# XiandaGuo/OpenStereo

Hardware: NVIDIA H100
Metric: stereo_pairs_per_sec_gwcnet_256x512_d192 (higher is better)
Workload: dtype f32

## Files before the change

openstereo_b200/csrc/conv3d_tc.cu:

```cuda
#include <cstdlib>
#include <type_traits>

#include "tc_common.cuh"

namespace osb {

constexpr int TC_W = 128;
constexpr int TC_KC = 32;
constexpr int TC_TILES = TC_WGS;
constexpr int TC_ROWS = TC_TILES + 2;
constexpr int TC_STAGES = 4;
constexpr int TC_RAW = 2;
constexpr int TC_ROW_BYTES = TC_W * TC_KC * 4;
constexpr int TC_PC = 16;

struct TcParams {
  const float* x;
  const void* w;
  const float* scale;
  const float* shift;
  const float* residual;
  float* y;
  int B, D, H, Cin, Cout;
  int act;
  float kappa;
  unsigned int* overflow;
  int out_ndhwc, res_ndhwc;
  int bulk_rows;
  int in_ncdhw;
  int items, hblocks;
};

template <int COUT>
struct TcCfg {
  static constexpr int N3 = 3 * COUT;
  static constexpr int B_SLICE = N3 * TC_KC * 4;
  static constexpr int NPASS = COUT / TC_PC;
  static constexpr int LD = 3 * TC_PC + 4;
  static constexpr int XCHG_FLOATS = 6 * 2 * TC_PC;
  static constexpr int A_OFF = 0;
  static constexpr int B_OFF = A_OFF + TC_STAGES * TC_ROW_BYTES;
  static constexpr int RAW_OFF = B_OFF + TC_BSLOTS * 3 * B_SLICE;
  static constexpr int STAGE_OFF = RAW_OFF + TC_RAW * TC_ROW_BYTES;
  static constexpr int BAR_OFF = STAGE_OFF + TC_WGS * 128 * LD * 4;
  static constexpr size_t SMEM = 1024 + (size_t)BAR_OFF + 256 + TC_WGS * XCHG_FLOATS * 4 + 2 * COUT * 4;
  static_assert(COUT % TC_PC == 0, "the epilogue stages whole passes of TC_PC channels");
  static_assert(B_SLICE % 1024 == 0, "weight slices must stay 1024-byte aligned");
  static_assert(32 * LD >= TP_WARP_FLOATS, "store_ndhwc_chunk32 transposes through the warp's own rows of the staging tile");
  static_assert(SMEM <= 232448, "shared memory budget of one CTA exceeded");
};

template <int COUT>
__device__ __forceinline__ void tc_stage_pass(float* stage, const float (&acc)[2][3 * COUT / 2], int pass, int wq, int lane) {
  constexpr int LD = TcCfg<COUT>::LD;
#pragma unroll
  for (int h = 0; h < 2; ++h) {
    float* r0 = stage + (64 * h + 16 * wq + (lane >> 2)) * LD + 2 * (lane & 3);
#pragma unroll
    for (int kw = 0; kw < 3; ++kw)
#pragma unroll
      for (int jj = 0; jj < TC_PC / 8; ++jj) {
        const int j = (kw * COUT + pass * TC_PC) / 8 + jj;
        *reinterpret_cast<float2*>(r0 + TC_PC * kw + 8 * jj) = make_float2(acc[h][4 * j], acc[h][4 * j + 1]);
        *reinterpret_cast<float2*>(r0 + 8 * LD + TC_PC * kw + 8 * jj) = make_float2(acc[h][4 * j + 2], acc[h][4 * j + 3]);
      }
  }
}

template <int COUT>
__global__ void __launch_bounds__(TC_WG_THREADS, 1) conv3d_tc_kernel(const TcParams p) {
  using C = TcCfg<COUT>;
  constexpr int N3 = C::N3;
  constexpr int B_SLICE = C::B_SLICE;
  extern __shared__ __align__(1024) uint8_t smem_raw[];
  uint8_t* smem = smem_raw + ((1024u - (smem_u32(smem_raw) & 1023u)) & 1023u);
  uint8_t* a_buf = smem + C::A_OFF;
  uint8_t* b_buf = smem + C::B_OFF;
  uint8_t* raw_buf = smem + C::RAW_OFF;
  float* stage = reinterpret_cast<float*>(smem + C::STAGE_OFF);
  uint64_t* bars = reinterpret_cast<uint64_t*>(smem + C::BAR_OFF);
  uint64_t* a_ready = bars;
  uint64_t* a_empty = a_ready + TC_STAGES;
  uint64_t* b_full = a_empty + TC_STAGES;
  uint64_t* b_empty = b_full + TC_BSLOTS * 3;
  uint64_t* raw_full = b_empty + TC_BSLOTS * 3;
  uint64_t* raw_empty = raw_full + TC_RAW;
  float* xchg = reinterpret_cast<float*>(smem + C::BAR_OFF + 256);
  float* s_scale = xchg + TC_WGS * C::XCHG_FLOATS;
  float* s_shift = s_scale + COUT;

  const int warp = threadIdx.x >> 5, lane = threadIdx.x & 31;
  const int nchunk = p.Cin / TC_KC;

  if (threadIdx.x == 0) {
    for (int s = 0; s < TC_STAGES; ++s) {
      mbar_init(&a_ready[s], 128);
      mbar_init(&a_empty[s], 4 * TC_WGS);
    }
    for (int k = 0; k < TC_BSLOTS * 3; ++k) {
      mbar_init(&b_full[k], 1);
      mbar_init(&b_empty[k], 4 * TC_WGS);
    }
    for (int k = 0; k < TC_RAW; ++k) {
      mbar_init(&raw_full[k], 1);
      mbar_init(&raw_empty[k], 128);
    }
    fence_mbar_init();
  }
  for (int c = threadIdx.x; c < COUT; c += blockDim.x) {
    s_scale[c] = p.scale ? p.scale[c] : 1.f;
    s_shift[c] = p.shift ? p.shift[c] : 0.f;
  }
  for (int i = threadIdx.x; i < TC_WGS * C::XCHG_FLOATS; i += blockDim.x) xchg[i] = 0.f;
  __syncthreads();
  struct RowIter {
    int it, kd, ch, r;
  };
  auto advance = [&](RowIter& s) {
    for (;;) {
      if (s.it >= p.items) return false;
      if (++s.r < TC_ROWS) return true;
      s.r = -1;
      if (++s.ch < nchunk) continue;
      s.ch = 0;
      const int d = (s.it / p.hblocks) % p.D;
      for (++s.kd; s.kd < 3; ++s.kd) {
        const int din = d + s.kd - 1;
        if (din >= 0 && din < p.D) break;
      }
      if (s.kd < 3) continue;
      s.it += gridDim.x;
      if (s.it >= p.items) return false;
      const int d2 = (s.it / p.hblocks) % p.D;
      s.kd = (d2 == 0) ? 1 : 0;
    }
  };
  if (warp < 4 * TC_WGS) {
    setmaxnreg_inc<TC_CONSUMER_REGS>();
    const int wg = warp >> 2;
    stage += wg * 128 * C::LD;
    xchg += wg * C::XCHG_FLOATS;
    const int bar_stage = 1 + 2 * wg, bar_xchg = 2 + 2 * wg;
    constexpr uint32_t LO = TcK<TC_KC>::LO_OFF;
    constexpr uint32_t A_HALF = 64 * TC_KC * 4 / 16;
    const uint64_t dbase = desc_sw128_base();
    const uint32_t b16 = (smem_u32(b_buf) & 0x3FFFF) >> 4;
    const int q = warp & 3;
    const int m = q * 32 + lane;
    uint32_t rowc = 0, phc = 0;
    for (int it = blockIdx.x; it < p.items; it += gridDim.x) {
      const int d = (it / p.hblocks) % p.D;
      float acc[2][N3 / 2];
      uint32_t accum = 0;
      for (int kd = 0; kd < 3; ++kd) {
        const int din = d + kd - 1;
        if (din < 0 || din >= p.D) continue;
        for (int ch = 0; ch < nchunk; ++ch, ++phc) {
          const uint32_t bslot = (phc & 1) * 3;
#pragma unroll
          for (int r = 0; r < TC_ROWS; ++r) {
            const uint32_t s = rowc % TC_STAGES, par = (rowc / TC_STAGES) & 1;
            mbar_wait(&a_ready[s], par);
            const int kh = r - wg;
            if (kh >= 0 && kh < 3) {
              mbar_wait(&b_full[bslot + kh], (phc >> 1) & 1);
              const uint64_t da0 = dbase | (uint64_t)((smem_u32(a_buf + s * TC_ROW_BYTES) & 0x3FFFF) >> 4);
              const uint64_t db0 = dbase | (uint64_t)(b16 + (bslot + kh) * (B_SLICE / 16));
              wg_fence();
#pragma unroll
              for (int ks = 0; ks < TcK<TC_KC>::KSTEPS; ++ks)
                wg_mma_split<N3>(acc, da0 + 2 * ks, A_HALF, db0 + 2 * ks, LO, ks > 0 ? 1u : accum);
              wg_commit();
              wg_wait_all();
              accum = 1;
              wg_release(&b_empty[bslot + kh], lane);
            }
            wg_release(&a_empty[s], lane);
            ++rowc;
          }
        }
      }
      const int h = (it % p.hblocks) * TC_TILES + wg;
      if (h >= p.H) continue;
      const float corr = 1.f + p.kappa * (float)(((d > 0) + 1 + (d + 1 < p.D)) * nchunk * 3 * TcK<TC_KC>::KSTEPS * 3);
      float out[COUT];
#pragma unroll
      for (int pass = 0; pass < C::NPASS; ++pass) {
        named_bar_sync(bar_stage, 128);
        tc_stage_pass<COUT>(stage, acc, pass, q, lane);
        named_bar_sync(bar_stage, 128);
        const float* srow = stage + m * C::LD;
        float* xq = xchg + (q + 1) * 2 * TC_PC;
        if (lane == 31) {
#pragma unroll
          for (int i = 0; i < TC_PC; i += 4)
            *reinterpret_cast<float4*>(xq + i) = *reinterpret_cast<const float4*>(srow + i);
        }
        if (lane == 0) {
#pragma unroll
          for (int i = 0; i < TC_PC; i += 4)
            *reinterpret_cast<float4*>(xq + TC_PC + i) = *reinterpret_cast<const float4*>(srow + 2 * TC_PC + i);
        }
        named_bar_sync(bar_xchg, 128);
        const float* xl = xq - 2 * TC_PC;
        const float* xr = xq + 3 * TC_PC;
#pragma unroll
        for (int i0 = 0; i0 < TC_PC; i0 += 4) {
          const float4 l4 = *reinterpret_cast<const float4*>(xl + i0);
          const float4 r4 = *reinterpret_cast<const float4*>(xr + i0);
          const float4 p04 = *reinterpret_cast<const float4*>(srow + i0);
          const float4 p14 = *reinterpret_cast<const float4*>(srow + TC_PC + i0);
          const float4 p24 = *reinterpret_cast<const float4*>(srow + 2 * TC_PC + i0);
          const float le[4] = {l4.x, l4.y, l4.z, l4.w}, re[4] = {r4.x, r4.y, r4.z, r4.w};
          const float p0[4] = {p04.x, p04.y, p04.z, p04.w}, p1[4] = {p14.x, p14.y, p14.z, p14.w}, p2[4] = {p24.x, p24.y, p24.z, p24.w};
#pragma unroll
          for (int k = 0; k < 4; ++k) {
            float left = __shfl_up_sync(0xffffffffu, p0[k], 1);
            float right = __shfl_down_sync(0xffffffffu, p2[k], 1);
            left = (lane == 0) ? le[k] : left;
            right = (lane == 31) ? re[k] : right;
            out[pass * TC_PC + i0 + k] = ((left + p1[k]) + right) * corr;
          }
        }
      }
      const int b = it / (p.hblocks * p.D);
      const size_t vox = (((size_t)b * p.D + d) * p.H + h) * TC_W + m;
      const size_t plane = (size_t)p.D * p.H * TC_W;
      const size_t ncdhw0 = (size_t)b * p.Cout * plane + ((size_t)d * p.H + h) * TC_W + m;
      if constexpr (COUT == 32) {
        if (p.out_ndhwc && (!p.residual || p.res_ndhwc)) {
          store_ndhwc_chunk32(stage + q * 32 * C::LD, lane, out, p.y + (vox - lane) * COUT,
                              p.residual ? p.residual + (vox - lane) * COUT : nullptr, COUT, s_scale, s_shift, p.act);
          continue;
        }
      }
#pragma unroll
      for (int i = 0; i < COUT; ++i) out[i] = fmaf(out[i], s_scale[i], s_shift[i]);
      if (p.residual) {
        if (p.res_ndhwc) {
          const float4* rp = reinterpret_cast<const float4*>(p.residual + vox * COUT);
#pragma unroll
          for (int i = 0; i < COUT / 4; ++i) {
            const float4 rv = __ldg(rp + i);
            out[4 * i] += rv.x, out[4 * i + 1] += rv.y, out[4 * i + 2] += rv.z, out[4 * i + 3] += rv.w;
          }
        } else {
#pragma unroll
          for (int i = 0; i < COUT; ++i)
            if (i < p.Cout) out[i] += __ldg(p.residual + ncdhw0 + (size_t)i * plane);
        }
      }
      if (p.act == OSB_ACT_RELU) {
#pragma unroll
        for (int i = 0; i < COUT; ++i) out[i] = fmaxf(out[i], 0.f);
      } else if (p.act == OSB_ACT_LEAKY) {
#pragma unroll
        for (int i = 0; i < COUT; ++i) out[i] = out[i] > 0.f ? out[i] : 0.01f * out[i];
      }
      if (p.out_ndhwc) {
        float4* yp = reinterpret_cast<float4*>(p.y + vox * COUT);
#pragma unroll
        for (int i = 0; i < COUT / 4; ++i) yp[i] = make_float4(out[4 * i], out[4 * i + 1], out[4 * i + 2], out[4 * i + 3]);
      } else {
#pragma unroll
        for (int i = 0; i < COUT; ++i)
          if (i < p.Cout) p.y[ncdhw0 + (size_t)i * plane] = out[i];
      }
    }
  }
  else if (warp < 4 * TC_WGS + 4) {
    setmaxnreg_dec<TC_LOADER_REGS>();
    const int lt = threadIdx.x - 4 * TC_WGS * 32;
    const int vsel = lt >> 3, c16 = lt & 7;
    const int vcol = ((vsel & 1) << 2) | ((vsel >> 1) & 3) | (vsel & 8);
    float amax = 0.f;
    auto run = [&](auto in_ncdhw) {
      constexpr bool NCDHW = decltype(in_ncdhw)::value;
      const size_t row_stride = (size_t)TC_W * p.Cin;
      auto load_row = [&](const RowIter& s, float4 (&v)[8]) {
        const int hb = s.it % p.hblocks;
        const int d = (s.it / p.hblocks) % p.D;
        const int b = s.it / (p.hblocks * p.D);
        const int hin = hb * TC_TILES - 1 + s.r, din = d + s.kd - 1;
        if (hin >= 0 && hin < p.H && NCDHW) {
          const size_t plane = (size_t)p.D * p.H * TC_W;
          const float* src = p.x + (((size_t)b * p.Cin + s.ch * TC_KC) * p.D + din) * p.H * TC_W + (size_t)hin * TC_W + lt;
#pragma unroll
          for (int j = 0; j < 8; ++j, src += 4 * plane)
            v[j] = make_float4(__ldg(src), __ldg(src + plane), __ldg(src + 2 * plane), __ldg(src + 3 * plane));
          const bool swap = (lt >> 3) & 1;
#pragma unroll
          for (int j = 0; j < 8; j += 2) {
            const float4 e = v[j], o = v[j + 1];
            v[j] = swap ? o : e;
            v[j + 1] = swap ? e : o;
          }
        } else if (hin >= 0 && hin < p.H) {
          const float* src = p.x + (((size_t)b * p.D + din) * p.H + hin) * row_stride + s.ch * TC_KC + c16 * 4 + vcol * p.Cin;
#pragma unroll
          for (int j = 0; j < 8; ++j) v[j] = __ldg(reinterpret_cast<const float4*>(src + 16 * j * p.Cin));
        } else {
#pragma unroll
          for (int j = 0; j < 8; ++j) v[j] = make_float4(0.f, 0.f, 0.f, 0.f);
        }
      };
      uint32_t rowc = 0;
      auto store_row = [&](const float4 (&v)[8]) {
        const uint32_t s = rowc % TC_STAGES, par = (rowc / TC_STAGES) & 1;
        mbar_wait_relaxed(&a_empty[s], par ^ 1);
        uint8_t* tile = a_buf + s * TC_ROW_BYTES;
        if (NCDHW) {
#pragma unroll
          for (int j = 0; j < 8; ++j) stage_f16_split<TC_KC>(tile, lt, j ^ ((lt >> 3) & 1), v[j], amax);
        } else {
#pragma unroll
          for (int j = 0; j < 8; ++j) stage_f16_split<TC_KC>(tile, vcol + 16 * j, c16, v[j], amax);
        }
        fence_proxy_async();
        mbar_arrive(&a_ready[s]);
        ++rowc;
      };
      RowIter ld{(int)blockIdx.x, 0, 0, -1};
      if (ld.it < p.items) ld.kd = (((ld.it / p.hblocks) % p.D) == 0) ? 1 : 0;
      if (p.bulk_rows) {
        uint32_t rawc = 0;
        while (advance(ld)) {
          const int hb = ld.it % p.hblocks;
          const int hin = hb * TC_TILES - 1 + ld.r;
          const uint32_t slot = rawc % TC_RAW, par = (rawc / TC_RAW) & 1;
          mbar_wait_relaxed(&raw_full[slot], par);
          float4 v[8];
          if (hin >= 0 && hin < p.H && NCDHW) {
            const float* src = reinterpret_cast<const float*>(raw_buf + slot * TC_ROW_BYTES) + lt;
#pragma unroll
            for (int j = 0; j < 8; ++j) {
              const float* q = src + 4 * (j ^ ((lt >> 3) & 1)) * TC_W;
              v[j] = make_float4(q[0], q[TC_W], q[2 * TC_W], q[3 * TC_W]);
            }
          } else if (hin >= 0 && hin < p.H) {
            const float* src = reinterpret_cast<const float*>(raw_buf + slot * TC_ROW_BYTES) + c16 * 4;
#pragma unroll
            for (int j = 0; j < 8; ++j) v[j] = *reinterpret_cast<const float4*>(src + (vcol + 16 * j) * TC_KC);
          } else {
#pragma unroll
            for (int j = 0; j < 8; ++j) v[j] = make_float4(0.f, 0.f, 0.f, 0.f);
          }
          store_row(v);
          mbar_arrive(&raw_empty[slot]);
          ++rawc;
        }
        tc_report_overflow(p.overflow, amax);
        amax = 0.f;
      }
      float4 va[8], vb[8];
      bool has_a = !p.bulk_rows && advance(ld);
      if (has_a) load_row(ld, va);
      bool has_b = has_a && advance(ld);
      if (has_b) load_row(ld, vb);
      while (has_a) {
        store_row(va);
        has_a = has_b && advance(ld);
        if (has_a) load_row(ld, va);
        if (!has_b) break;
        store_row(vb);
        has_b = has_a && advance(ld);
        if (has_b) load_row(ld, vb);
      }
      tc_report_overflow(p.overflow, amax);
    };
    if (p.in_ncdhw) run(std::true_type{});
    else run(std::false_type{});
  }
  else {
    setmaxnreg_dec<TC_PRODUCER_REGS>();
    if (warp == 4 * TC_WGS + 4 && elect_one()) {
      const uint8_t* wsrc = reinterpret_cast<const uint8_t*>(p.w);
      uint32_t phc = 0;
      for (int it = blockIdx.x; it < p.items; it += gridDim.x) {
        const int d = (it / p.hblocks) % p.D;
        for (int kd = 0; kd < 3; ++kd) {
          const int din = d + kd - 1;
          if (din < 0 || din >= p.D) continue;
          for (int ch = 0; ch < nchunk; ++ch, ++phc) {
            for (int kh = 0; kh < 3; ++kh) {
              const uint32_t slot = (phc & 1) * 3 + kh;
              const size_t slice = ((size_t)kd * nchunk + ch) * 3 + kh;
              mbar_wait_relaxed(&b_empty[slot], ((phc >> 1) & 1) ^ 1);
              mbar_arrive_expect_tx(&b_full[slot], B_SLICE);
              bulk_g2s(b_buf + slot * B_SLICE, wsrc + slice * B_SLICE, B_SLICE, &b_full[slot]);
            }
          }
        }
      }
    }
    else if (warp == 4 * TC_WGS + 5 && p.bulk_rows && elect_one()) {
      RowIter ld{(int)blockIdx.x, 0, 0, -1};
      if (ld.it < p.items) ld.kd = (((ld.it / p.hblocks) % p.D) == 0) ? 1 : 0;
      uint32_t rawc = 0;
      while (advance(ld)) {
        const int hb = ld.it % p.hblocks;
        const int d = (ld.it / p.hblocks) % p.D;
        const int b = ld.it / (p.hblocks * p.D);
        const int hin = hb * TC_TILES - 1 + ld.r, din = d + ld.kd - 1;
        const uint32_t slot = rawc % TC_RAW, par = (rawc / TC_RAW) & 1;
        mbar_wait_relaxed(&raw_empty[slot], par ^ 1);
        if (hin >= 0 && hin < p.H && p.in_ncdhw) {
          const size_t plane = (size_t)p.D * p.H * TC_W;
          const float* src = p.x + (((size_t)b * p.Cin + ld.ch * TC_KC) * p.D + din) * p.H * TC_W + (size_t)hin * TC_W;
          mbar_arrive_expect_tx(&raw_full[slot], TC_ROW_BYTES);
          for (int c = 0; c < TC_KC; ++c)
            bulk_g2s(raw_buf + slot * TC_ROW_BYTES + c * (TC_W * 4), src + c * plane, TC_W * 4, &raw_full[slot]);
        } else if (hin >= 0 && hin < p.H) {
          const float* src = p.x + (((size_t)b * p.D + din) * p.H + hin) * (size_t)(TC_W * TC_KC);
          mbar_arrive_expect_tx(&raw_full[slot], TC_ROW_BYTES);
          bulk_g2s(raw_buf + slot * TC_ROW_BYTES, src, TC_ROW_BYTES, &raw_full[slot]);
        } else {
          mbar_arrive(&raw_full[slot]);
        }
        ++rawc;
      }
    }
    __syncwarp();
  }
}

__global__ void __launch_bounds__(256) ncdhw_to_ndhwc_kernel(const float* __restrict__ x, float* __restrict__ y, int C, int Cp,
                                                             size_t vol) {
  __shared__ float tile[32][33];
  const int b = blockIdx.z;
  const size_t v0 = (size_t)blockIdx.x * 32;
  const int c0 = blockIdx.y * 32;
  const int tx = threadIdx.x & 31, ty = threadIdx.x >> 5;
  for (int i = ty; i < 32; i += 8) {
    const int c = c0 + i;
    const size_t v = v0 + tx;
    tile[i][tx] = (c < C && v < vol) ? __ldg(x + ((size_t)b * C + c) * vol + v) : 0.f;
  }
  __syncthreads();
  for (int i = ty; i < 32; i += 8) {
    const size_t v = v0 + i;
    const int c = c0 + tx;
    if (c < Cp && v < vol) y[((size_t)b * vol + v) * Cp + c] = tile[tx][i];
  }
}

template <int COUT>
static int launch_tc(const TcParams& p, cudaStream_t stream) {
  const size_t smem = TcCfg<COUT>::SMEM;
  auto kernel = conv3d_tc_kernel<COUT>;
  static PerDeviceFlag configured;
  if (!configured.here()) {
    cudaError_t e = cudaFuncSetAttribute(kernel, cudaFuncAttributeMaxDynamicSharedMemorySize, (int)smem);
    if (e != cudaSuccess) {
      set_error("conv3d_tc: cannot reserve %zu bytes of shared memory: %s", smem, cudaGetErrorString(e));
      return OSB_ECUDA;
    }
    configured.here() = true;
  }
  const int sms = sm_count();
  const int grid = (int)cap_persistent_grid(p.items < sms ? p.items : sms);
  static const std::string variant = tc_variant_name("tc<%d>", COUT);
  set_tc_variant(variant.c_str());
  kernel<<<grid, TC_WG_THREADS, smem, stream>>>(p);
  count_launch();
  return check_launch("conv3d_tc_kernel");
}

int launch_tcg_dispatch(const float* x, const void* w, const float* scale, const float* shift, const float* residual, float* y,
                        int B, int Cin, int Cout, int D, int H, int W, int act, int out_ndhwc, int res_ndhwc, cudaStream_t stream,
                        const float* gate = nullptr, int ystride = 0);
int launch_tcg_dilated2(const float* x, const void* w, const float* scale, const float* shift, const float* residual, float* y,
                        int B, int Cin, int Cout, int H, int W, int act, int out_ndhwc, int res_ndhwc, cudaStream_t stream);

}

extern "C" {

int osb_tc_general_width(int W) { return W >= OSB_TC_MIN_WIDTH ? 1 : 0; }

int osb_conv3d_tc_kc(int Cin, int Cout, int W, int stride) {
  if (stride != 1) return 0;
  if (W == osb::TC_W && (Cout == 32 || (Cout >= 1 && Cout <= 16)) && Cin % 32 == 0 && Cin >= 32) return 32;
  if (Cin % 16 == 0 && Cin >= 16 &&
      ((W == 64 && Cout == 64) || (W == 32 && (Cout == 64 || Cout == 96 || Cout == 128)) || (W == 16 && (Cout == 64 || Cout == 96)) ||
       (W == osb::TC_W && (Cout == 64 || Cout == 128))))
    return 16;
  if (Cin % 16 == 0 && Cin >= 16 && osb_tc_general_width(W) && (Cout == 32 || Cout == 64 || Cout == 128))
    return 16;
  return 0;
}

int osb_conv3d_tc_supported(int Cin, int Cout, int W, int stride) { return osb_conv3d_tc_kc(Cin, Cout, W, stride) != 0; }

int osb_ncdhw_to_ndhwc_pad(const float* x, float* y, int B, int C, int Cpad, int D, int H, int W, osb_stream_t stream) {
  using namespace osb;
  OSB_REQUIRE(x && y, "ncdhw_to_ndhwc: null pointer");
  OSB_REQUIRE(B > 0 && C > 0 && Cpad >= C && D > 0 && H > 0 && W > 0 && B <= 65535, "ncdhw_to_ndhwc: bad shape");
  const size_t vol = (size_t)D * H * W;
  dim3 grid((unsigned)((vol + 31) / 32), (Cpad + 31) / 32, B);
  ncdhw_to_ndhwc_kernel<<<grid, 256, 0, (cudaStream_t)stream>>>(x, y, C, Cpad, vol);
  count_launch();
  return check_launch("ncdhw_to_ndhwc_kernel");
}

int osb_ncdhw_to_ndhwc(const float* x, float* y, int B, int C, int D, int H, int W, osb_stream_t stream) {
  return osb_ncdhw_to_ndhwc_pad(x, y, B, C, C, D, H, W, stream);
}

static int conv3d_k3_tc_impl(const float* x_ndhwc, const void* w_split, const float* scale, const float* shift,
                             const float* residual, float* y, int B, int Cin, int Cout, int D, int H, int W, int act,
                             int out_ndhwc, int res_ndhwc, int in_ncdhw, osb_stream_t stream, const float* gate = nullptr,
                             int ystride = 0) {
  using namespace osb;
  OSB_REQUIRE(x_ndhwc && w_split && y, "conv3d_k3_tc: null pointer");
  OSB_REQUIRE(B > 0 && D > 0 && H > 0, "conv3d_k3_tc: empty shape");
  OSB_REQUIRE(osb_conv3d_tc_supported(Cin, Cout, W, 1), "conv3d_k3_tc: unsupported shape Cin=%d Cout=%d W=%d", Cin, Cout, W);
  OSB_REQUIRE(act >= 0 && act <= 2, "conv3d_k3_tc: unknown activation %d", act);
  OSB_REQUIRE((reinterpret_cast<uintptr_t>(x_ndhwc) & 15) == 0 && (reinterpret_cast<uintptr_t>(w_split) & 15) == 0 &&
                  (reinterpret_cast<uintptr_t>(y) & 15) == 0 && (reinterpret_cast<uintptr_t>(residual) & 15) == 0,
              "conv3d_k3_tc: pointers must be 16-byte aligned");
  OSB_REQUIRE(!in_ncdhw || osb_conv3d_tc_kc(Cin, Cout, W, 1) == 32, "conv3d_k3_tc: NCDHW input is served by the W = 128 kernel only");
  OSB_REQUIRE(ystride == 0 || (ystride >= Cout && ystride % 4 == 0 && osb_conv3d_tc_kc(Cin, Cout, W, 1) == 16 && out_ndhwc &&
                                (!residual || res_ndhwc)),
              "conv3d_k3_tc: a channel slice (ystride %d) needs channels-last tensors on the 16-channel-chunk kernels", ystride);
  OSB_REQUIRE(!gate || (osb_conv3d_tc_kc(Cin, Cout, W, 1) == 16 && out_ndhwc && (!residual || res_ndhwc) &&
                        (reinterpret_cast<uintptr_t>(gate) & 15) == 0),
              "conv3d_k3_tc: the gate operand needs a channels-last output (and residual) on the 16-channel-chunk kernels");
  if (osb_conv3d_tc_kc(Cin, Cout, W, 1) == 16)
    return launch_tcg_dispatch(x_ndhwc, w_split, scale, shift, residual, y, B, Cin, Cout, D, H, W, act, out_ndhwc, res_ndhwc,
                               (cudaStream_t)stream, gate, ystride);
  TcParams p{};
  p.x = x_ndhwc, p.w = w_split, p.scale = scale, p.shift = shift, p.residual = residual, p.y = y;
  p.B = B, p.D = D, p.H = H, p.Cin = Cin, p.Cout = Cout, p.act = act;
  p.kappa = rz_kappa(), p.overflow = tc_overflow_flag();
  OSB_REQUIRE(p.overflow, "conv3d_k3_tc: cannot allocate the overflow flag");
  p.out_ndhwc = out_ndhwc, p.res_ndhwc = res_ndhwc, p.in_ncdhw = in_ncdhw;
  {
    static const int bulk = [] { const char* e = getenv("OSB_TC_BULK"); return e ? atoi(e) : 1; }();
    p.bulk_rows = (bulk && (in_ncdhw || Cin == TC_KC)) ? 1 : 0;
  }
  p.hblocks = (H + TC_TILES - 1) / TC_TILES;
  const long long items = (long long)B * D * p.hblocks;
  OSB_REQUIRE(items < (1ll << 31), "conv3d_k3_tc: too many work items");
  p.items = (int)items;
  if (Cout <= 16) {
    OSB_REQUIRE(!out_ndhwc && (!residual || !res_ndhwc), "conv3d_k3_tc: Cout <= 16 writes (and adds) NCDHW tensors only");
    return launch_tc<16>(p, (cudaStream_t)stream);
  }
  return launch_tc<32>(p, (cudaStream_t)stream);
}

int osb_conv3d_k3_tc_fwd(const float* x_ndhwc, const void* w_split, const float* scale, const float* shift,
                         const float* residual, float* y, int B, int Cin, int Cout, int D, int H, int W, int act,
                         int out_ndhwc, int res_ndhwc, osb_stream_t stream) {
  return conv3d_k3_tc_impl(x_ndhwc, w_split, scale, shift, residual, y, B, Cin, Cout, D, H, W, act, out_ndhwc, res_ndhwc, 0, stream);
}

int osb_conv3d_k3_tc_gate_fwd(const float* x_ndhwc, const void* w_split, const float* scale, const float* shift,
                              const float* residual, const float* gate_nhwc, float* y, int B, int Cin, int Cout, int D, int H, int W,
                              int act, osb_stream_t stream) {
  OSB_REQUIRE(gate_nhwc, "conv3d_k3_tc_gate: null gate");
  return conv3d_k3_tc_impl(x_ndhwc, w_split, scale, shift, residual, y, B, Cin, Cout, D, H, W, act, 1, 1, 0, stream, gate_nhwc);
}

int osb_conv3d_k3_tc_cs_fwd(const float* x_ndhwc, const void* w_split, const float* scale, const float* shift, const float* residual,
                            const float* gate_nhwc, float* y, int B, int Cin, int Cout, int D, int H, int W, int act, int ystride,
                            osb_stream_t stream) {
  return conv3d_k3_tc_impl(x_ndhwc, w_split, scale, shift, residual, y, B, Cin, Cout, D, H, W, act, 1, 1, 0, stream, gate_nhwc, ystride);
}

int osb_conv3d_k3_tc_ncdhw_fwd(const float* x_ncdhw, const void* w_split, const float* scale, const float* shift,
                               const float* residual, float* y, int B, int Cin, int Cout, int D, int H, int W, int act,
                               int out_ndhwc, int res_ndhwc, osb_stream_t stream) {
  return conv3d_k3_tc_impl(x_ncdhw, w_split, scale, shift, residual, y, B, Cin, Cout, D, H, W, act, out_ndhwc, res_ndhwc, 1, stream);
}

int osb_conv2d_tc_kc(int Cin, int Cout, int W, int dilation) {
  if (dilation == 1) return osb_conv3d_tc_kc(Cin, Cout, W, 1);
  if (dilation == 2 && W == osb::TC_W && Cout == 128 && Cin % 16 == 0 && Cin >= 16) return 16;
  return 0;
}

int osb_conv2d_k3_tc_fwd(const float* x_nhwc, const void* w_split, const float* scale, const float* shift, const float* residual,
                         float* y, int B, int Cin, int Cout, int H, int W, int dilation, int act, int out_nhwc, int res_nhwc,
                         osb_stream_t stream) {
  using namespace osb;
  if (dilation == 1)
    return osb_conv3d_k3_tc_fwd(x_nhwc, w_split, scale, shift, residual, y, B, Cin, Cout, 1, H, W, act, out_nhwc, res_nhwc, stream);
  OSB_REQUIRE(x_nhwc && w_split && y, "conv2d_k3_tc: null pointer");
  OSB_REQUIRE(B > 0 && H > 0, "conv2d_k3_tc: empty shape");
  OSB_REQUIRE(osb_conv2d_tc_kc(Cin, Cout, W, dilation) != 0, "conv2d_k3_tc: unsupported shape Cin=%d Cout=%d W=%d dilation=%d", Cin, Cout,
              W, dilation);
  OSB_REQUIRE(act >= 0 && act <= 2, "conv2d_k3_tc: unknown activation %d", act);
  OSB_REQUIRE((reinterpret_cast<uintptr_t>(x_nhwc) & 15) == 0 && (reinterpret_cast<uintptr_t>(w_split) & 15) == 0 &&
                  (reinterpret_cast<uintptr_t>(y) & 15) == 0 && (reinterpret_cast<uintptr_t>(residual) & 15) == 0,
              "conv2d_k3_tc: pointers must be 16-byte aligned");
  return launch_tcg_dilated2(x_nhwc, w_split, scale, shift, residual, y, B, Cin, Cout, H, W, act, out_nhwc, res_nhwc,
                             (cudaStream_t)stream);
}
}
```

openstereo_b200/csrc/conv3d_tcg.cu:

```cuda
#include "tc_common.cuh"

namespace osb {

struct TcgParams {
  const float* x;
  const void* w;
  const float* scale;
  const float* shift;
  const float* residual;
  const float* gate;
  float* y;
  int B, D, H, Cin;
  int act;
  float kappa;
  unsigned int* overflow;
  int out_ndhwc, res_ndhwc;
  int items, hblocks;
  int Wr, ctiles;
  int ystride;
};

template <int COUT, int KC, int W, int TILES, int DIL = 1, bool GW = false>
struct TcgCfg {
  static_assert(!GW || W == 128, "general-width tiles are 128-column segments of one image row");
  static constexpr int HALO = GW ? DIL : 0;
  static constexpr int CSTEP = 128 - 2 * HALO;
  static_assert(DIL == 1 || (W == 128 && DIL == 2 && COUT >= 64), "dilation 2 is instantiated for full-width rows only");
  static constexpr int R = 128 / W;
  static constexpr int ROWB = KC * 4;
  static constexpr int UNIT_BYTES = 128 * ROWB;
  static constexpr int N3 = 3 * COUT;
  static constexpr int G = 32;
  static constexpr int NG = COUT / G;
  static constexpr int NG3 = 3 * G;
  static constexpr int B_SLICE = N3 * ROWB;
  static constexpr int B_SUB = NG3 * ROWB;
  static constexpr int LD = NG3 + 4;
  static constexpr int NT = TC_WGS * TILES;
  static constexpr int TS = R * DIL;
  static constexpr int HSPAN = NT * TS;
  __host__ __device__ static constexpr int row0(int hb) { return (hb / DIL) * HSPAN + (hb % DIL) * R; }
  __host__ static int hblocks(int H) { return DIL * ((H + HSPAN - 1) / HSPAN); }
  static constexpr int NLW = 4;
  static constexpr int XCHG_FLOATS = 2 * 4 * 2 * DIL * 32;
  static constexpr int FIXED_SMEM = 1024 + TC_BSLOTS * 3 * B_SUB + TC_WGS * 128 * LD * 4 + 1024 + TC_WGS * XCHG_FLOATS * 4 + 3 * COUT * 4;
  static constexpr int STAGES = (232448 - FIXED_SMEM) / UNIT_BYTES < 10 ? (232448 - FIXED_SMEM) / UNIT_BYTES : 10;
  static_assert(STAGES >= NLW, "the ring must hold at least one unit per loader warp");
  static constexpr int S_FIRST = -DIL;
  static constexpr int S_LAST = (NT - 1) * TS + DIL;
  static constexpr int KSTEPS = KC / 16;
  static constexpr int LO = KC / 8;
  static constexpr int A_OFF = 0;
  static constexpr int B_OFF = A_OFF + STAGES * UNIT_BYTES;
  static constexpr int STAGE_OFF = B_OFF + TC_BSLOTS * 3 * B_SUB;
  static constexpr int BAR_OFF = STAGE_OFF + TC_WGS * 128 * LD * 4;
  static constexpr int THREADS = TC_WG_THREADS;
  static constexpr size_t SMEM = 1024 + (size_t)BAR_OFF + 1024 + TC_WGS * XCHG_FLOATS * 4 + 3 * COUT * 4;
  static_assert(SMEM <= 232448, "shared memory budget of one CTA exceeded");
  static_assert(TILES == 1, "a consumer warpgroup holds one accumulator tile");
  static_assert(DIL == 1 || R == 1, "interleaved row blocks assume one image row per tile");
  static_assert(COUT % G == 0, "output channels come in groups of 32");
  static_assert(B_SUB % 1024 == 0 && UNIT_BYTES % 1024 == 0, "operand tiles must stay 1024-byte aligned");
  static constexpr int tile_of(int s, int kh) {
    const int num = s - (kh - 1) * DIL;
    return (num >= 0 && num % TS == 0 && num / TS < NT) ? num / TS : -1;
  }
  static constexpr bool used(int s) { return tile_of(s, 0) >= 0 || tile_of(s, 1) >= 0 || tile_of(s, 2) >= 0; }
  static constexpr int units_per_phase() {
    int n = 0;
    for (int s = S_FIRST; s <= S_LAST; ++s) n += used(s) ? 1 : 0;
    return n;
  }
  static constexpr int NU = units_per_phase();
  static constexpr int unit_s(int j) {
    int k = 0;
    for (int s = S_FIRST; s <= S_LAST; ++s)
      if (used(s)) {
        if (k == j) return s;
        ++k;
      }
    return S_LAST;
  }
};

template <int COUT, int KC, int W, int TILES, int DIL = 1, bool GW = false, bool GATE = false>
__global__ void __launch_bounds__(TcgCfg<COUT, KC, W, TILES, DIL, GW>::THREADS, 1) conv3d_tcg_kernel(const TcgParams p) {
  using C = TcgCfg<COUT, KC, W, TILES, DIL, GW>;
  extern __shared__ __align__(1024) uint8_t smem_raw[];
  uint8_t* smem = reinterpret_cast<uint8_t*>((reinterpret_cast<uintptr_t>(smem_raw) + 1023) & ~static_cast<uintptr_t>(1023));
  uint8_t* a_buf = smem + C::A_OFF;
  uint8_t* b_buf = smem + C::B_OFF;
  float* stage = reinterpret_cast<float*>(smem + C::STAGE_OFF);
  uint64_t* bars = reinterpret_cast<uint64_t*>(smem + C::BAR_OFF);
  uint64_t* a_ready = bars;
  uint64_t* a_empty = a_ready + C::STAGES;
  uint64_t* b_full = a_empty + C::STAGES;
  uint64_t* b_empty = b_full + TC_BSLOTS * 3;
  float* xchg = reinterpret_cast<float*>(smem + C::BAR_OFF + 1024);
  float* s_scale = xchg + TC_WGS * C::XCHG_FLOATS;
  float* s_shift = s_scale + COUT;
  float* zeros = s_shift + COUT;

  const int warp = threadIdx.x >> 5, lane = threadIdx.x & 31;
  const int nchunk = p.Cin / KC;
  const int Wp = GW ? p.Wr : W;
  const int YS = (W < 32 && p.ystride) ? p.ystride : COUT;
  const int ctiles = GW ? p.ctiles : 1;

  if (threadIdx.x == 0) {
    for (int s = 0; s < C::STAGES; ++s) {
      mbar_init(&a_ready[s], 32);
      mbar_init(&a_empty[s], 4 * TC_WGS);
    }
    for (int k = 0; k < TC_BSLOTS * 3; ++k) {
      mbar_init(&b_full[k], 1);
      mbar_init(&b_empty[k], 4 * TC_WGS);
    }
    fence_mbar_init();
  }
  for (int c = threadIdx.x; c < COUT; c += blockDim.x) {
    s_scale[c] = p.scale ? p.scale[c] : 1.f;
    s_shift[c] = p.shift ? p.shift[c] : 0.f;
    zeros[c] = 0.f;
  }
  __syncthreads();

  if (warp < 4 * TC_WGS) {
    setmaxnreg_inc<TC_CONSUMER_REGS>();
    const int wg = warp >> 2;
    stage += wg * 128 * C::LD;
    xchg += wg * C::XCHG_FLOATS;
    const int bar_stage = 1 + 2 * wg, bar_xchg = 2 + 2 * wg;
    const uint64_t dbase = (KC == 32) ? desc_sw128_base() : desc_sw64_base();
    constexpr uint32_t A_HALF = 64 * C::ROWB / 16;
    const uint32_t b16 = (smem_u32(b_buf) & 0x3FFFF) >> 4;
    const int q = warp & 3;
    const int m = q * 32 + lane;
    const int rr = m / W, wcol = m % W;
    const bool has_left_q = ((q * 32) % W) != 0;
    const bool has_right_q = (((q + 1) * 32) % W) != 0;
    uint32_t unitc = 0, phc = 0, exc = 0;
    for (int it = blockIdx.x; it < p.items; it += gridDim.x) {
      const int cg = (it % C::NG) * C::G;
      const int it0 = it / C::NG;
      const int ct = it0 % ctiles;
      const int hb = (it0 / ctiles) % p.hblocks;
      const int d = (it0 / (ctiles * p.hblocks)) % p.D;
      const int b = it0 / (ctiles * p.hblocks * p.D);
      {
        float acc[2][C::NG3 / 2];
        uint32_t accum = 0;
        for (int kd = 0; kd < 3; ++kd) {
          const int din = d + kd - 1;
          if (din < 0 || din >= p.D) continue;
          for (int ch = 0; ch < nchunk; ++ch, ++phc) {
#pragma unroll
            for (int s = C::S_FIRST; s <= C::S_LAST; ++s) {
              if (!C::used(s)) continue;
              const uint32_t slot = unitc % C::STAGES, par = (unitc / C::STAGES) & 1;
              mbar_wait(&a_ready[slot], par);
              const uint64_t da0 = dbase | (uint64_t)((smem_u32(a_buf + slot * C::UNIT_BYTES) & 0x3FFFF) >> 4);
#pragma unroll
              for (int kh = 0; kh < 3; ++kh) {
                if (C::tile_of(s, kh) != wg) continue;
                const uint32_t bslot = (phc & 1) * 3 + kh;
                mbar_wait(&b_full[bslot], (phc >> 1) & 1);
                const uint64_t db0 = dbase | (uint64_t)(b16 + (bslot * C::B_SUB) / 16);
                wg_fence();
#pragma unroll
                for (int ks = 0; ks < C::KSTEPS; ++ks)
                  wg_mma_split<C::NG3>(acc, da0 + 2 * ks, A_HALF, db0 + 2 * ks, C::LO, ks > 0 ? 1u : accum);
                wg_commit();
                wg_wait_all();
                accum = 1;
                wg_release(&b_empty[bslot], lane);
              }
              wg_release(&a_empty[slot], lane);
              ++unitc;
            }
          }
        }
        named_bar_sync(bar_stage, 128);
        wg_stage<C::NG3>(stage, C::LD, acc, q, lane);
        named_bar_sync(bar_stage, 128);
      }
      const int col = GW ? ct * C::CSTEP - C::HALO + m : wcol;
      const bool cvalid = !GW || (m >= C::HALO && m < 128 - C::HALO && col < Wp);
      const uint32_t vmask = GW ? __ballot_sync(0xffffffffu, cvalid) : 0xffffffffu;
      const float corr = 1.f + p.kappa * (float)(((d > 0) + 1 + (d + 1 < p.D)) * nchunk * 3 * C::KSTEPS * 3);
      {
        const int h = C::row0(hb) + wg * C::TS + rr;
        const bool live = h < p.H;
        const ptrdiff_t vox = (((ptrdiff_t)b * p.D + d) * p.H + h) * Wp + col;
        if (live && cvalid && p.residual && p.res_ndhwc) {
          const float* rp = p.residual + vox * YS;
#pragma unroll
          for (int k = 0; k < COUT; k += 32) asm volatile("prefetch.global.L2 [%0];" ::"l"(rp + k));
        }
        const size_t plane = (size_t)p.D * p.H * Wp;
        const ptrdiff_t ncdhw0 = (ptrdiff_t)b * COUT * plane + ((ptrdiff_t)d * p.H + h) * Wp + col;
        {
          const float* srow = stage + m * C::LD;
          float* xb = xchg + (exc & 1) * (4 * 2 * DIL * 32);
          ++exc;
          if (lane >= 32 - DIL) {
#pragma unroll
            for (int i = 0; i < 32; i += 4)
              *reinterpret_cast<float4*>(xb + ((q * 2) * DIL + lane - (32 - DIL)) * 32 + i) = *reinterpret_cast<const float4*>(srow + i);
          }
          if (lane < DIL) {
#pragma unroll
            for (int i = 0; i < 32; i += 4)
              *reinterpret_cast<float4*>(xb + ((q * 2 + 1) * DIL + lane) * 32 + i) = *reinterpret_cast<const float4*>(srow + 2 * C::G + i);
          }
          named_bar_sync(bar_xchg, 128);
          const float* xl = has_left_q ? xb + (((q - 1) * 2) * DIL + (lane < DIL ? lane : 0)) * 32 : zeros;
          const float* xr = has_right_q ? xb + (((q + 1) * 2 + 1) * DIL + (lane >= 32 - DIL ? lane - (32 - DIL) : 0)) * 32 : zeros;
          float out[32];
#pragma unroll
          for (int i0 = 0; i0 < 32; i0 += 4) {
            const float4 l4 = *reinterpret_cast<const float4*>(xl + i0);
            const float4 r4 = *reinterpret_cast<const float4*>(xr + i0);
            const float4 p04 = *reinterpret_cast<const float4*>(srow + i0);
            const float4 p14 = *reinterpret_cast<const float4*>(srow + C::G + i0);
            const float4 p24 = *reinterpret_cast<const float4*>(srow + 2 * C::G + i0);
            const float le[4] = {l4.x, l4.y, l4.z, l4.w}, re[4] = {r4.x, r4.y, r4.z, r4.w};
            const float p0[4] = {p04.x, p04.y, p04.z, p04.w}, p1[4] = {p14.x, p14.y, p14.z, p14.w}, p2[4] = {p24.x, p24.y, p24.z, p24.w};
#pragma unroll
            for (int k = 0; k < 4; ++k) {
              const int i = i0 + k;
              float left = __shfl_up_sync(0xffffffffu, p0[k], DIL);
              float right = __shfl_down_sync(0xffffffffu, p2[k], DIL);
              left = (lane < DIL) ? le[k] : left;
              right = (lane >= 32 - DIL) ? re[k] : right;
              if (W < 32) {
                left = (wcol < DIL) ? 0.f : left;
                right = (wcol >= W - DIL) ? 0.f : right;
              }
              out[i] = ((left + p1[k]) + right) * corr;
            }
          }
          const uint32_t vm = (W < 32) ? __ballot_sync(0xffffffffu, live) : (live ? vmask : 0u);
          if (vm && p.out_ndhwc && (!p.residual || p.res_ndhwc)) {
            const ptrdiff_t gvox = GATE ? ((ptrdiff_t)b * p.H + h) * Wp + col - lane : 0;
            store_ndhwc_chunk32(stage + q * 32 * C::LD, lane, out, p.y + (vox - lane) * YS + cg,
                                p.residual ? p.residual + (vox - lane) * YS + cg : nullptr, YS, s_scale + cg, s_shift + cg, p.act,
                                vm, (GATE && p.gate) ? p.gate + gvox * YS + cg : nullptr);
          } else if (live && cvalid) {
#pragma unroll
            for (int i = 0; i < 32; ++i) out[i] = fmaf(out[i], s_scale[cg + i], s_shift[cg + i]);
            if (p.residual) {
              if (p.res_ndhwc) {
                const float4* rp = reinterpret_cast<const float4*>(p.residual + vox * YS + cg);
#pragma unroll
                for (int i = 0; i < 8; ++i) {
                  const float4 rv = __ldg(rp + i);
                  out[4 * i] += rv.x, out[4 * i + 1] += rv.y, out[4 * i + 2] += rv.z, out[4 * i + 3] += rv.w;
                }
              } else {
#pragma unroll
                for (int i = 0; i < 32; ++i) out[i] += __ldg(p.residual + ncdhw0 + (size_t)(cg + i) * plane);
              }
            }
            if (p.act == OSB_ACT_RELU) {
#pragma unroll
              for (int i = 0; i < 32; ++i) out[i] = fmaxf(out[i], 0.f);
            } else if (p.act == OSB_ACT_LEAKY) {
#pragma unroll
              for (int i = 0; i < 32; ++i) out[i] = out[i] > 0.f ? out[i] : 0.01f * out[i];
            }
            if (p.out_ndhwc) {
              float4* yp = reinterpret_cast<float4*>(p.y + vox * YS + cg);
#pragma unroll
              for (int i = 0; i < 8; ++i) yp[i] = make_float4(out[4 * i], out[4 * i + 1], out[4 * i + 2], out[4 * i + 3]);
            } else {
#pragma unroll
              for (int i = 0; i < 32; ++i) p.y[ncdhw0 + (size_t)(cg + i) * plane] = out[i];
            }
          }
        }
      }
    }
  }
  else if (warp < 4 * TC_WGS + C::NLW) {
    setmaxnreg_dec<TC_LOADER_REGS>();
    const int lw = warp - 4 * TC_WGS;
    static_assert(KC == 16, "lane_voxel / unit-row mapping below is written for 64-byte operand rows");
    constexpr int CPR = KC / 4;
    constexpr int VPL = 32 / CPR;
    constexpr int NLD = 128 / VPL;
    static_assert(W % VPL == 0, "a load instruction must not straddle image rows");
    const int v0 = lane_voxel<KC>(lane), c = lane % CPR;
    float amax = 0.f;
    uint32_t ubase = 0;
    int first = lw;
    auto fill = [&](const float* base, size_t rstride, size_t cstride, int h_first, int h_step, uint32_t u, int col0) {
      float4 v[NLD];
#pragma unroll
      for (int j = 0; j < NLD; ++j) {
        const int hin = h_first + h_step * ((VPL * j) / W);
        const size_t off = (size_t)((VPL * j) / W) * rstride + (size_t)((VPL * j) % W) * cstride;
        bool ok = hin >= 0 && hin < p.H;
        if (GW) ok = ok && (unsigned)(col0 + VPL * j) < (unsigned)Wp;
        v[j] = ok ? __ldg(reinterpret_cast<const float4*>(base + (ptrdiff_t)off)) : make_float4(0.f, 0.f, 0.f, 0.f);
      }
      const uint32_t slot = u % C::STAGES, ph = (u / C::STAGES) & 1;
      mbar_wait_relaxed(&a_empty[slot], ph ^ 1);
      uint8_t* tile = a_buf + slot * C::UNIT_BYTES;
#pragma unroll
      for (int j = 0; j < NLD; ++j) stage_f16_split<KC>(tile, v0 + VPL * j, c, v[j], amax);
      fence_proxy_async();
      mbar_arrive(&a_ready[slot]);
    };
    for (int it = blockIdx.x; it < p.items; it += gridDim.x) {
      const int it0 = it / C::NG;
      const int ct = it0 % ctiles;
      const int hb = (it0 / ctiles) % p.hblocks;
      const int d = (it0 / (ctiles * p.hblocks)) % p.D;
      const int b = it0 / (ctiles * p.hblocks * p.D);
      const int h0 = C::row0(hb);
      const int col0 = ct * C::CSTEP - C::HALO + v0;
      for (int kd = 0; kd < 3; ++kd) {
        const int din = d + kd - 1;
        if (din < 0 || din >= p.D) continue;
        const float* plane = p.x + ((size_t)b * p.D + din) * p.H * (size_t)Wp * p.Cin;
        for (int ch = 0; ch < nchunk; ++ch) {
#pragma unroll 1
          for (int j = first; j < C::NU; j += C::NLW) {
            const int s = C::unit_s(j);
            const float* base = plane + ((ptrdiff_t)(h0 + s) * Wp + col0) * p.Cin + ch * KC + c * 4;
            fill(base, (size_t)Wp * p.Cin, (size_t)p.Cin, h0 + s, 1, ubase + j, col0);
          }
          ubase += C::NU;
          first = (first + C::NLW - C::NU % C::NLW) % C::NLW;
        }
      }
    }
    tc_report_overflow(p.overflow, amax);
  }
  else {
    setmaxnreg_dec<TC_PRODUCER_REGS>();
    if (warp == 4 * TC_WGS + C::NLW && elect_one()) {
      const uint8_t* wsrc = reinterpret_cast<const uint8_t*>(p.w);
      uint32_t phc = 0;
      for (int it = blockIdx.x; it < p.items; it += gridDim.x) {
        const int cg = (it % C::NG) * C::G;
        const int d = (it / C::NG / (ctiles * p.hblocks)) % p.D;
        for (int kd = 0; kd < 3; ++kd) {
          const int din = d + kd - 1;
          if (din < 0 || din >= p.D) continue;
          for (int ch = 0; ch < nchunk; ++ch, ++phc) {
            for (int kh = 0; kh < 3; ++kh) {
              const uint32_t slot = (phc & 1) * 3 + kh;
              const size_t slice = ((size_t)kd * nchunk + ch) * 3 + kh;
              mbar_wait_relaxed(&b_empty[slot], ((phc >> 1) & 1) ^ 1);
              mbar_arrive_expect_tx(&b_full[slot], C::B_SUB);
#pragma unroll
              for (int kw = 0; kw < 3; ++kw)
                bulk_g2s(b_buf + slot * C::B_SUB + kw * C::G * C::ROWB, wsrc + slice * C::B_SLICE + (size_t)(kw * COUT + cg) * C::ROWB,
                         C::G * C::ROWB, &b_full[slot]);
            }
          }
        }
      }
    }
    __syncwarp();
  }
}

template <int COUT, int KC, int W, int TILES, int DIL = 1, bool GW = false, bool GATE = false>
static int launch_tcg(TcgParams& p, cudaStream_t stream) {
  using C = TcgCfg<COUT, KC, W, TILES, DIL, GW>;
  auto kernel = conv3d_tcg_kernel<COUT, KC, W, TILES, DIL, GW, GATE>;
  if (!GATE && p.gate) {
    set_error("conv3d_tcg: no gated instantiation for Cout=%d W=%d", COUT, W);
    return OSB_EUNSUPPORTED;
  }
  if (W >= 32 && p.ystride && p.ystride != COUT) {
    set_error("conv3d_tcg: channel slices are instantiated for W = 16 only");
    return OSB_EUNSUPPORTED;
  }
  static PerDeviceFlag configured;
  if (!configured.here()) {
    cudaError_t e = cudaFuncSetAttribute(kernel, cudaFuncAttributeMaxDynamicSharedMemorySize, (int)C::SMEM);
    if (e != cudaSuccess) {
      set_error("conv3d_tcg: cannot reserve %zu bytes of shared memory: %s", C::SMEM, cudaGetErrorString(e));
      return OSB_ECUDA;
    }
    configured.here() = true;
  }
  p.hblocks = C::hblocks(p.H);
  if (GW) p.ctiles = (p.Wr + C::CSTEP - 1) / C::CSTEP;
  else p.Wr = W, p.ctiles = 1;
  const long long items = (long long)p.B * p.D * p.hblocks * p.ctiles * C::NG;
  OSB_REQUIRE(items < (1ll << 31), "conv3d_tcg: too many work items");
  p.items = (int)items;
  const int sms = sm_count();
  const int grid = (int)cap_persistent_grid(p.items < sms ? p.items : sms);
  static const std::string variant = tc_variant_name("tcg<%d,%d,%d,%d,%d,%d,%d>", COUT, KC, W, TILES, DIL, (int)GW, (int)GATE);
  set_tc_variant(variant.c_str());
  kernel<<<grid, C::THREADS, C::SMEM, stream>>>(p);
  count_launch();
  cudaError_t le = cudaGetLastError();
  if (le != cudaSuccess) {
    cudaFuncAttributes fa{};
    (void)cudaFuncGetAttributes(&fa, kernel);
    set_error("conv3d_tcg_kernel<%d,%d,%d,%d>: launch failed: %s (threads %d, kernel maxThreadsPerBlock %d, regs %d, static smem %zu, "
              "dynamic smem %zu, max dynamic %d)", COUT, KC, W, TILES, cudaGetErrorString(le), C::THREADS, fa.maxThreadsPerBlock,
              fa.numRegs, fa.sharedSizeBytes, C::SMEM, fa.maxDynamicSharedSizeBytes);
    return OSB_ECUDA;
  }
  return OSB_OK;
}

int launch_tcg_dispatch(const float* x, const void* w, const float* scale, const float* shift, const float* residual, float* y,
                        int B, int Cin, int Cout, int D, int H, int W, int act, int out_ndhwc, int res_ndhwc, cudaStream_t stream,
                        const float* gate, int ystride) {
  TcgParams p{};
  p.x = x, p.w = w, p.scale = scale, p.shift = shift, p.residual = residual, p.y = y, p.gate = gate;
  p.ystride = ystride;
  p.B = B, p.D = D, p.H = H, p.Cin = Cin, p.act = act, p.out_ndhwc = out_ndhwc, p.res_ndhwc = res_ndhwc;
  p.kappa = rz_kappa(), p.overflow = tc_overflow_flag();
  if (!p.overflow) return OSB_ECUDA;
  if (Cin % 16 != 0 || Cin < 16) return -1;
  if (W == 64 && Cout == 64 && gate) return launch_tcg<64, 16, 64, 1, 1, false, true>(p, stream);
  if (W == 32 && Cout == 96 && gate) return launch_tcg<96, 16, 32, 1, 1, false, true>(p, stream);
  if (W == 64 && Cout == 64) return launch_tcg<64, 16, 64, 1>(p, stream);
  if (W == 32 && Cout == 64) return launch_tcg<64, 16, 32, 1>(p, stream);
  if (W == 32 && Cout == 128) return launch_tcg<128, 16, 32, 1>(p, stream);
  if (W == 32 && Cout == 96) return launch_tcg<96, 16, 32, 1>(p, stream);
  if (W == 16 && Cout == 96) return launch_tcg<96, 16, 16, 1, 1, false, true>(p, stream);
  if (W == 16 && Cout == 64) return launch_tcg<64, 16, 16, 1, 1, false, true>(p, stream);
  if (W == 128 && Cout == 64) return launch_tcg<64, 16, 128, 1>(p, stream);
  if (W == 128 && Cout == 128) return launch_tcg<128, 16, 128, 1>(p, stream);
  p.Wr = W;
  if (Cout == 32) return launch_tcg<32, 16, 128, 1, 1, true>(p, stream);
  if (Cout == 64) return launch_tcg<64, 16, 128, 1, 1, true>(p, stream);
  if (Cout == 128) return launch_tcg<128, 16, 128, 1, 1, true>(p, stream);
  return -1;
}

int launch_tcg_dilated2(const float* x, const void* w, const float* scale, const float* shift, const float* residual, float* y,
                        int B, int Cin, int Cout, int H, int W, int act, int out_ndhwc, int res_ndhwc, cudaStream_t stream) {
  TcgParams p{};
  p.x = x, p.w = w, p.scale = scale, p.shift = shift, p.residual = residual, p.y = y;
  p.B = B, p.D = 1, p.H = H, p.Cin = Cin, p.act = act, p.out_ndhwc = out_ndhwc, p.res_ndhwc = res_ndhwc;
  p.kappa = rz_kappa(), p.overflow = tc_overflow_flag();
  if (!p.overflow) return OSB_ECUDA;
  if (Cin % 16 != 0 || Cin < 16) return -1;
  if (W == 128 && Cout == 128) return launch_tcg<128, 16, 128, 1, 2>(p, stream);
  return -1;
}

}
```

openstereo_b200/csrc/tc_common.cuh:

```cuda
#pragma once
#include "common.cuh"

namespace osb {

__device__ __forceinline__ void mbar_wait_relaxed(uint64_t* bar, uint32_t parity) {
  uint32_t done;
  for (;;) {
    asm volatile(
        "{\n.reg .pred p;\nmbarrier.try_wait.parity.shared::cta.b64 p, [%1], %2;\nselp.u32 %0, 1, 0, p;\n}\n"
        : "=r"(done)
        : "r"(smem_u32(bar)), "r"(parity)
        : "memory");
    if (done) return;
    __nanosleep(64);
  }
}
__device__ __forceinline__ void mbar_arrive(uint64_t* bar) {
  asm volatile("mbarrier.arrive.shared::cta.b64 _, [%0];" ::"r"(smem_u32(bar)) : "memory");
}
__device__ __forceinline__ uint64_t desc_sw128_base() {
  uint64_t d = 0;
  d |= (uint64_t)1 << 16;
  d |= (uint64_t)(1024 >> 4) << 32;
  d |= (uint64_t)1 << 62;
  return d;
}
__device__ __forceinline__ uint64_t desc_sw64_base() {
  uint64_t d = 0;
  d |= (uint64_t)1 << 16;
  d |= (uint64_t)(512 >> 4) << 32;
  d |= (uint64_t)2 << 62;
  return d;
}

template <int N>
__device__ __forceinline__ void wgmma_f16(float (&d)[N / 2], uint64_t da, uint64_t db, uint32_t accumulate);
template <>
__device__ __forceinline__ void wgmma_f16<32>(float (&d)[16], uint64_t da, uint64_t db, uint32_t accumulate) {
  asm volatile(
      "{\n.reg .pred p;\nsetp.ne.b32 p, %18, 0;\n"
      "wgmma.mma_async.sync.aligned.m64n32k16.f32.f16.f16 {%0, %1, %2, %3, %4, %5, %6, %7, %8, %9, %10, %11, %12, %13, %14, %15}, %16, %17, p, 1, 1, 0, 0;\n}\n"
      : "+f"(d[0]), "+f"(d[1]), "+f"(d[2]), "+f"(d[3]), "+f"(d[4]), "+f"(d[5]), "+f"(d[6]), "+f"(d[7]), "+f"(d[8]), "+f"(d[9]), "+f"(d[10]), "+f"(d[11]), "+f"(d[12]), "+f"(d[13]), "+f"(d[14]), "+f"(d[15])
      : "l"(da), "l"(db), "r"(accumulate)
      : "memory");
}

template <>
__device__ __forceinline__ void wgmma_f16<48>(float (&d)[24], uint64_t da, uint64_t db, uint32_t accumulate) {
  asm volatile(
      "{\n.reg .pred p;\nsetp.ne.b32 p, %26, 0;\n"
      "wgmma.mma_async.sync.aligned.m64n48k16.f32.f16.f16 {%0, %1, %2, %3, %4, %5, %6, %7, %8, %9, %10, %11, %12, %13, %14, %15, %16, %17, %18, %19, %20, %21, %22, %23}, %24, %25, p, 1, 1, 0, 0;\n}\n"
      : "+f"(d[0]), "+f"(d[1]), "+f"(d[2]), "+f"(d[3]), "+f"(d[4]), "+f"(d[5]), "+f"(d[6]), "+f"(d[7]), "+f"(d[8]), "+f"(d[9]), "+f"(d[10]), "+f"(d[11]), "+f"(d[12]), "+f"(d[13]), "+f"(d[14]), "+f"(d[15]), "+f"(d[16]), "+f"(d[17]), "+f"(d[18]), "+f"(d[19]), "+f"(d[20]), "+f"(d[21]), "+f"(d[22]), "+f"(d[23])
      : "l"(da), "l"(db), "r"(accumulate)
      : "memory");
}

template <>
__device__ __forceinline__ void wgmma_f16<64>(float (&d)[32], uint64_t da, uint64_t db, uint32_t accumulate) {
  asm volatile(
      "{\n.reg .pred p;\nsetp.ne.b32 p, %34, 0;\n"
      "wgmma.mma_async.sync.aligned.m64n64k16.f32.f16.f16 {%0, %1, %2, %3, %4, %5, %6, %7, %8, %9, %10, %11, %12, %13, %14, %15, %16, %17, %18, %19, %20, %21, %22, %23, %24, %25, %26, %27, %28, %29, %30, %31}, %32, %33, p, 1, 1, 0, 0;\n}\n"
      : "+f"(d[0]), "+f"(d[1]), "+f"(d[2]), "+f"(d[3]), "+f"(d[4]), "+f"(d[5]), "+f"(d[6]), "+f"(d[7]), "+f"(d[8]), "+f"(d[9]), "+f"(d[10]), "+f"(d[11]), "+f"(d[12]), "+f"(d[13]), "+f"(d[14]), "+f"(d[15]), "+f"(d[16]), "+f"(d[17]), "+f"(d[18]), "+f"(d[19]), "+f"(d[20]), "+f"(d[21]), "+f"(d[22]), "+f"(d[23]), "+f"(d[24]), "+f"(d[25]), "+f"(d[26]), "+f"(d[27]), "+f"(d[28]), "+f"(d[29]), "+f"(d[30]), "+f"(d[31])
      : "l"(da), "l"(db), "r"(accumulate)
      : "memory");
}

template <>
__device__ __forceinline__ void wgmma_f16<96>(float (&d)[48], uint64_t da, uint64_t db, uint32_t accumulate) {
  asm volatile(
      "{\n.reg .pred p;\nsetp.ne.b32 p, %50, 0;\n"
      "wgmma.mma_async.sync.aligned.m64n96k16.f32.f16.f16 {%0, %1, %2, %3, %4, %5, %6, %7, %8, %9, %10, %11, %12, %13, %14, %15, %16, %17, %18, %19, %20, %21, %22, %23, %24, %25, %26, %27, %28, %29, %30, %31, %32, %33, %34, %35, %36, %37, %38, %39, %40, %41, %42, %43, %44, %45, %46, %47}, %48, %49, p, 1, 1, 0, 0;\n}\n"
      : "+f"(d[0]), "+f"(d[1]), "+f"(d[2]), "+f"(d[3]), "+f"(d[4]), "+f"(d[5]), "+f"(d[6]), "+f"(d[7]), "+f"(d[8]), "+f"(d[9]), "+f"(d[10]), "+f"(d[11]), "+f"(d[12]), "+f"(d[13]), "+f"(d[14]), "+f"(d[15]), "+f"(d[16]), "+f"(d[17]), "+f"(d[18]), "+f"(d[19]), "+f"(d[20]), "+f"(d[21]), "+f"(d[22]), "+f"(d[23]), "+f"(d[24]), "+f"(d[25]), "+f"(d[26]), "+f"(d[27]), "+f"(d[28]), "+f"(d[29]), "+f"(d[30]), "+f"(d[31]), "+f"(d[32]), "+f"(d[33]), "+f"(d[34]), "+f"(d[35]), "+f"(d[36]), "+f"(d[37]), "+f"(d[38]), "+f"(d[39]), "+f"(d[40]), "+f"(d[41]), "+f"(d[42]), "+f"(d[43]), "+f"(d[44]), "+f"(d[45]), "+f"(d[46]), "+f"(d[47])
      : "l"(da), "l"(db), "r"(accumulate)
      : "memory");
}

template <>
__device__ __forceinline__ void wgmma_f16<128>(float (&d)[64], uint64_t da, uint64_t db, uint32_t accumulate) {
  asm volatile(
      "{\n.reg .pred p;\nsetp.ne.b32 p, %66, 0;\n"
      "wgmma.mma_async.sync.aligned.m64n128k16.f32.f16.f16 {%0, %1, %2, %3, %4, %5, %6, %7, %8, %9, %10, %11, %12, %13, %14, %15, %16, %17, %18, %19, %20, %21, %22, %23, %24, %25, %26, %27, %28, %29, %30, %31, %32, %33, %34, %35, %36, %37, %38, %39, %40, %41, %42, %43, %44, %45, %46, %47, %48, %49, %50, %51, %52, %53, %54, %55, %56, %57, %58, %59, %60, %61, %62, %63}, %64, %65, p, 1, 1, 0, 0;\n}\n"
      : "+f"(d[0]), "+f"(d[1]), "+f"(d[2]), "+f"(d[3]), "+f"(d[4]), "+f"(d[5]), "+f"(d[6]), "+f"(d[7]), "+f"(d[8]), "+f"(d[9]), "+f"(d[10]), "+f"(d[11]), "+f"(d[12]), "+f"(d[13]), "+f"(d[14]), "+f"(d[15]), "+f"(d[16]), "+f"(d[17]), "+f"(d[18]), "+f"(d[19]), "+f"(d[20]), "+f"(d[21]), "+f"(d[22]), "+f"(d[23]), "+f"(d[24]), "+f"(d[25]), "+f"(d[26]), "+f"(d[27]), "+f"(d[28]), "+f"(d[29]), "+f"(d[30]), "+f"(d[31]), "+f"(d[32]), "+f"(d[33]), "+f"(d[34]), "+f"(d[35]), "+f"(d[36]), "+f"(d[37]), "+f"(d[38]), "+f"(d[39]), "+f"(d[40]), "+f"(d[41]), "+f"(d[42]), "+f"(d[43]), "+f"(d[44]), "+f"(d[45]), "+f"(d[46]), "+f"(d[47]), "+f"(d[48]), "+f"(d[49]), "+f"(d[50]), "+f"(d[51]), "+f"(d[52]), "+f"(d[53]), "+f"(d[54]), "+f"(d[55]), "+f"(d[56]), "+f"(d[57]), "+f"(d[58]), "+f"(d[59]), "+f"(d[60]), "+f"(d[61]), "+f"(d[62]), "+f"(d[63])
      : "l"(da), "l"(db), "r"(accumulate)
      : "memory");
}

__device__ __forceinline__ void wg_fence() { asm volatile("wgmma.fence.sync.aligned;" ::: "memory"); }
__device__ __forceinline__ void wg_commit() { asm volatile("wgmma.commit_group.sync.aligned;" ::: "memory"); }
__device__ __forceinline__ void wg_wait_all() { asm volatile("wgmma.wait_group.sync.aligned 0;" ::: "memory"); }

template <int N>
__device__ __forceinline__ void wg_mma_split(float (&acc)[2][N / 2], uint64_t da, uint32_t a_half, uint64_t db, uint32_t lo,
                                             uint32_t accumulate) {
#pragma unroll
  for (int h = 0; h < 2; ++h) {
    wgmma_f16<N>(acc[h], da + h * a_half + lo, db, accumulate);
    wgmma_f16<N>(acc[h], da + h * a_half, db + lo, 1);
    wgmma_f16<N>(acc[h], da + h * a_half, db, 1);
  }
}
__device__ __forceinline__ void wg_release(uint64_t* bar, int lane) {
  if (lane == 0) mbar_arrive(bar);
}
template <int N>
__device__ __forceinline__ void wg_stage(float* stage, int ld, const float (&acc)[2][N / 2], int wq, int lane) {
#pragma unroll
  for (int h = 0; h < 2; ++h) {
    float* r0 = stage + (64 * h + 16 * wq + (lane >> 2)) * ld + 2 * (lane & 3);
#pragma unroll
    for (int j = 0; j < N / 8; ++j) {
      *reinterpret_cast<float2*>(r0 + 8 * j) = make_float2(acc[h][4 * j], acc[h][4 * j + 1]);
      *reinterpret_cast<float2*>(r0 + 8 * ld + 8 * j) = make_float2(acc[h][4 * j + 2], acc[h][4 * j + 3]);
    }
  }
}
__device__ __forceinline__ void stage_ld16(const float* row, uint32_t* r) {
#pragma unroll
  for (int i = 0; i < 4; ++i) {
    const float4 v = reinterpret_cast<const float4*>(row)[i];
    r[4 * i] = __float_as_uint(v.x), r[4 * i + 1] = __float_as_uint(v.y), r[4 * i + 2] = __float_as_uint(v.z), r[4 * i + 3] = __float_as_uint(v.w);
  }
}

__device__ __forceinline__ void bulk_g2s(void* smem_dst, const void* gsrc, uint32_t bytes, uint64_t* bar) {
  asm volatile("cp.async.bulk.shared::cluster.global.mbarrier::complete_tx::bytes [%0], [%1], %2, [%3];" ::"r"(smem_u32(smem_dst)),
               "l"(gsrc), "r"(bytes), "r"(smem_u32(bar))
               : "memory");
}
__device__ __forceinline__ void cp_async16(void* smem_dst, const void* gsrc, bool valid) {
  const uint32_t n = valid ? 16u : 0u;
  asm volatile("cp.async.ca.shared.global [%0], [%1], 16, %2;" ::"r"(smem_u32(smem_dst)), "l"(gsrc), "r"(n) : "memory");
}
__device__ __forceinline__ void cp_async_commit() { asm volatile("cp.async.commit_group;" ::: "memory"); }
template <int N>
__device__ __forceinline__ void cp_async_wait() {
  asm volatile("cp.async.wait_group %0;" ::"n"(N) : "memory");
}
constexpr int TC_BSLOTS = 2;
__device__ __forceinline__ void named_bar_sync(int id, int threads) {
  asm volatile("bar.sync %0, %1;" ::"r"(id), "r"(threads) : "memory");
}
__device__ __forceinline__ void named_bar_arrive(int id, int threads) {
  asm volatile("bar.arrive %0, %1;" ::"r"(id), "r"(threads) : "memory");
}
constexpr int TC_WGS = 2;
constexpr int TC_CONSUMER_REGS = 184;
constexpr int TC_LOADER_REGS = 112;
constexpr int TC_PRODUCER_REGS = 32;
constexpr int TC_WG_THREADS = 512;
template <int N>
__device__ __forceinline__ void setmaxnreg_inc() {
  asm volatile("setmaxnreg.inc.sync.aligned.u32 %0;" ::"n"(N));
}
template <int N>
__device__ __forceinline__ void setmaxnreg_dec() {
  asm volatile("setmaxnreg.dec.sync.aligned.u32 %0;" ::"n"(N));
}
__device__ __forceinline__ bool elect_one() {
  uint32_t pred;
  asm volatile("{\n.reg .pred p;\nelect.sync _|p, 0xffffffff;\nselp.u32 %0, 1, 0, p;\n}\n" : "=r"(pred));
  return pred != 0;
}
constexpr float TC_ACT_SCALE = 16.f;
constexpr float TC_F16_MAX = 65504.f;
__device__ __forceinline__ uint32_t cvt_f16x2_sat(float a, float b) {
  uint32_t r;
  asm("cvt.rn.satfinite.f16x2.f32 %0, %1, %2;" : "=r"(r) : "f"(b), "f"(a));
  return r;
}
__device__ __forceinline__ float2 f16x2_to_float2(uint32_t h) {
  float2 f;
  asm("{\n.reg .b16 l, u;\nmov.b32 {l, u}, %2;\ncvt.f32.f16 %0, l;\ncvt.f32.f16 %1, u;\n}\n" : "=f"(f.x), "=f"(f.y) : "r"(h));
  return f;
}
__device__ __forceinline__ void f16_split4(const float4 v, uint2& hi, uint2& lo, float& amax) {
  const float x0 = v.x * TC_ACT_SCALE, x1 = v.y * TC_ACT_SCALE, x2 = v.z * TC_ACT_SCALE, x3 = v.w * TC_ACT_SCALE;
  amax = fmaxf(amax, fmaxf(fmaxf(fabsf(x0), fabsf(x1)), fmaxf(fabsf(x2), fabsf(x3))));
  hi.x = cvt_f16x2_sat(x0, x1);
  hi.y = cvt_f16x2_sat(x2, x3);
  const float2 h01 = f16x2_to_float2(hi.x), h23 = f16x2_to_float2(hi.y);
  lo.x = cvt_f16x2_sat(x0 - h01.x, x1 - h01.y);
  lo.y = cvt_f16x2_sat(x2 - h23.x, x3 - h23.y);
}
unsigned int* tc_overflow_flag();
__device__ __forceinline__ void tc_report_overflow(unsigned int* flag, float amax) {
  if (amax > TC_F16_MAX) atomicAdd(flag, 1u);
}

float rz_kappa();


template <int KC>
__device__ __forceinline__ int swz_offset(int row, int c) {
  if constexpr (KC == 32) return row * 128 + ((c ^ (row & 7)) << 4);
  else return row * 64 + ((c ^ ((row >> 1) & 3)) << 4);
}


template <int KC>
__device__ __forceinline__ void stage_f16_split(uint8_t* tile, int row, int q, const float4 v, float& amax) {
  uint2 hi, lo;
  f16_split4(v, hi, lo, amax);
  const int sub = (q & 1) << 3;
  *reinterpret_cast<uint2*>(tile + swz_offset<KC>(row, q >> 1) + sub) = hi;
  *reinterpret_cast<uint2*>(tile + swz_offset<KC>(row, KC / 8 + (q >> 1)) + sub) = lo;
}
template <int KC>
__device__ __forceinline__ int lane_voxel(int lane) {
  if constexpr (KC == 32) return (((lane >> 3) & 1) << 2) | (lane >> 4);
  else return ((lane >> 2) & 1) | (((lane >> 3) & 1) << 2) | ((lane >> 4) << 1);
}
template <int KC>
struct TcK {
  static constexpr int KSTEPS = KC / 16;
  static constexpr int LO_OFF = KC / 8;
};

constexpr int TP_STRIDE = 36;
constexpr int TP_WARP_FLOATS = 32 * TP_STRIDE;

__device__ __forceinline__ void store_ndhwc_chunk32(float* tbuf, int lane, const float (&sum)[32], float* y0, const float* res0,
                                                    size_t vstride, const float* sc, const float* sh, int act,
                                                    uint32_t vmask = 0xffffffffu, const float* gate0 = nullptr) {
  const int c4 = 4 * (lane & 7), sub = lane >> 3;
  __syncwarp();
  float4* row = reinterpret_cast<float4*>(tbuf + lane * TP_STRIDE);
#pragma unroll
  for (int i = 0; i < 8; ++i) row[i] = make_float4(sum[4 * i], sum[4 * i + 1], sum[4 * i + 2], sum[4 * i + 3]);
  __syncwarp();
  const float4 a = *reinterpret_cast<const float4*>(sc + c4);
  const float4 b = *reinterpret_cast<const float4*>(sh + c4);
  float4 o[8];
#pragma unroll
  for (int j = 0; j < 8; ++j) {
    o[j] = *reinterpret_cast<const float4*>(tbuf + (4 * j + sub) * TP_STRIDE + c4);
    o[j].x = fmaf(o[j].x, a.x, b.x), o[j].y = fmaf(o[j].y, a.y, b.y), o[j].z = fmaf(o[j].z, a.z, b.z), o[j].w = fmaf(o[j].w, a.w, b.w);
  }
  if (res0) {
    float4 r[8];
#pragma unroll
    for (int j = 0; j < 8; ++j)
      r[j] = ((vmask >> (4 * j + sub)) & 1u) ? __ldg(reinterpret_cast<const float4*>(res0 + (size_t)(4 * j + sub) * vstride + c4))
                                             : make_float4(0.f, 0.f, 0.f, 0.f);
#pragma unroll
    for (int j = 0; j < 8; ++j) o[j].x += r[j].x, o[j].y += r[j].y, o[j].z += r[j].z, o[j].w += r[j].w;
  }
  if (act == OSB_ACT_RELU) {
#pragma unroll
    for (int j = 0; j < 8; ++j) o[j].x = fmaxf(o[j].x, 0.f), o[j].y = fmaxf(o[j].y, 0.f), o[j].z = fmaxf(o[j].z, 0.f), o[j].w = fmaxf(o[j].w, 0.f);
  } else if (act == OSB_ACT_LEAKY) {
#pragma unroll
    for (int j = 0; j < 8; ++j) {
      o[j].x = o[j].x > 0.f ? o[j].x : 0.01f * o[j].x, o[j].y = o[j].y > 0.f ? o[j].y : 0.01f * o[j].y;
      o[j].z = o[j].z > 0.f ? o[j].z : 0.01f * o[j].z, o[j].w = o[j].w > 0.f ? o[j].w : 0.01f * o[j].w;
    }
  }
  if (gate0) {
#pragma unroll
    for (int j = 0; j < 8; ++j) {
      if (!((vmask >> (4 * j + sub)) & 1u)) continue;
      const float4 g = __ldg(reinterpret_cast<const float4*>(gate0 + (size_t)(4 * j + sub) * vstride + c4));
      o[j].x *= g.x, o[j].y *= g.y, o[j].z *= g.z, o[j].w *= g.w;
    }
  }
#pragma unroll
  for (int j = 0; j < 8; ++j)
    if ((vmask >> (4 * j + sub)) & 1u) *reinterpret_cast<float4*>(y0 + (size_t)(4 * j + sub) * vstride + c4) = o[j];
}

}
```

Baseline: 265.7.

## Compute conv3d epilogue directly on wgmma fragments instead of staging through shared memory

Replaces the per-pass staging of the full 3*COUT accumulator tile through a large shared-memory buffer with a register-level kw-unshift. The unshift uses warp shuffles and a small halo exchange buffer, and is followed by a fragment-based epilogue that transposes only small per-warp tiles for coalesced NDHWC stores. The change also adds an L2 prefetch of residual and gate rows before the MMA loop, and frees the staging shared memory (more ring stages in tcg). It is meant to cut shared-memory traffic and named-barrier syncs in the epilogue. In exchange, the boundary and wrap logic becomes more complex and more error-prone.

```diff
diff --git a/openstereo_b200/csrc/conv3d_tc.cu b/openstereo_b200/csrc/conv3d_tc.cu
--- a/openstereo_b200/csrc/conv3d_tc.cu
+++ b/openstereo_b200/csrc/conv3d_tc.cu
@@ -12,7 +12,6 @@
 constexpr int TC_STAGES = 4;
 constexpr int TC_RAW = 2;
 constexpr int TC_ROW_BYTES = TC_W * TC_KC * 4;
-constexpr int TC_PC = 16;
 
 struct TcParams {
   const float* x;
@@ -35,37 +34,15 @@
 struct TcCfg {
   static constexpr int N3 = 3 * COUT;
   static constexpr int B_SLICE = N3 * TC_KC * 4;
-  static constexpr int NPASS = COUT / TC_PC;
-  static constexpr int LD = 3 * TC_PC + 4;
-  static constexpr int XCHG_FLOATS = 6 * 2 * TC_PC;
+  static constexpr int XCHG_FLOATS = 2 * frag_xchg_floats<COUT, 1>();
   static constexpr int A_OFF = 0;
   static constexpr int B_OFF = A_OFF + TC_STAGES * TC_ROW_BYTES;
   static constexpr int RAW_OFF = B_OFF + TC_BSLOTS * 3 * B_SLICE;
-  static constexpr int STAGE_OFF = RAW_OFF + TC_RAW * TC_ROW_BYTES;
-  static constexpr int BAR_OFF = STAGE_OFF + TC_WGS * 128 * LD * 4;
-  static constexpr size_t SMEM = 1024 + (size_t)BAR_OFF + 256 + TC_WGS * XCHG_FLOATS * 4 + 2 * COUT * 4;
-  static_assert(COUT % TC_PC == 0, "the epilogue stages whole passes of TC_PC channels");
+  static constexpr int BAR_OFF = RAW_OFF + TC_RAW * TC_ROW_BYTES;
+  static constexpr size_t SMEM = 1024 + (size_t)BAR_OFF + 256 + TC_WGS * XCHG_FLOATS * 4 + 4 * TC_WGS * FRAG_TP_FLOATS * 4 + 2 * COUT * 4;
   static_assert(B_SLICE % 1024 == 0, "weight slices must stay 1024-byte aligned");
-  static_assert(32 * LD >= TP_WARP_FLOATS, "store_ndhwc_chunk32 transposes through the warp's own rows of the staging tile");
   static_assert(SMEM <= 232448, "shared memory budget of one CTA exceeded");
 };
-
-template <int COUT>
-__device__ __forceinline__ void tc_stage_pass(float* stage, const float (&acc)[2][3 * COUT / 2], int pass, int wq, int lane) {
-  constexpr int LD = TcCfg<COUT>::LD;
-#pragma unroll
-  for (int h = 0; h < 2; ++h) {
-    float* r0 = stage + (64 * h + 16 * wq + (lane >> 2)) * LD + 2 * (lane & 3);
-#pragma unroll
-    for (int kw = 0; kw < 3; ++kw)
-#pragma unroll
-      for (int jj = 0; jj < TC_PC / 8; ++jj) {
-        const int j = (kw * COUT + pass * TC_PC) / 8 + jj;
-        *reinterpret_cast<float2*>(r0 + TC_PC * kw + 8 * jj) = make_float2(acc[h][4 * j], acc[h][4 * j + 1]);
-        *reinterpret_cast<float2*>(r0 + 8 * LD + TC_PC * kw + 8 * jj) = make_float2(acc[h][4 * j + 2], acc[h][4 * j + 3]);
-      }
-  }
-}
 
 template <int COUT>
 __global__ void __launch_bounds__(TC_WG_THREADS, 1) conv3d_tc_kernel(const TcParams p) {
@@ -77,7 +54,6 @@
   uint8_t* a_buf = smem + C::A_OFF;
   uint8_t* b_buf = smem + C::B_OFF;
   uint8_t* raw_buf = smem + C::RAW_OFF;
-  float* stage = reinterpret_cast<float*>(smem + C::STAGE_OFF);
   uint64_t* bars = reinterpret_cast<uint64_t*>(smem + C::BAR_OFF);
   uint64_t* a_ready = bars;
   uint64_t* a_empty = a_ready + TC_STAGES;
@@ -86,7 +62,8 @@
   uint64_t* raw_full = b_empty + TC_BSLOTS * 3;
   uint64_t* raw_empty = raw_full + TC_RAW;
   float* xchg = reinterpret_cast<float*>(smem + C::BAR_OFF + 256);
-  float* s_scale = xchg + TC_WGS * C::XCHG_FLOATS;
+  float* tiles = xchg + TC_WGS * C::XCHG_FLOATS;
+  float* s_scale = tiles + 4 * TC_WGS * FRAG_TP_FLOATS;
   float* s_shift = s_scale + COUT;
 
   const int warp = threadIdx.x >> 5, lane = threadIdx.x & 31;
@@ -111,7 +88,6 @@
     s_scale[c] = p.scale ? p.scale[c] : 1.f;
     s_shift[c] = p.shift ? p.shift[c] : 0.f;
   }
-  for (int i = threadIdx.x; i < TC_WGS * C::XCHG_FLOATS; i += blockDim.x) xchg[i] = 0.f;
   __syncthreads();
   struct RowIter {
     int it, kd, ch, r;
@@ -138,18 +114,20 @@
   if (warp < 4 * TC_WGS) {
     setmaxnreg_inc<TC_CONSUMER_REGS>();
     const int wg = warp >> 2;
-    stage += wg * 128 * C::LD;
     xchg += wg * C::XCHG_FLOATS;
-    const int bar_stage = 1 + 2 * wg, bar_xchg = 2 + 2 * wg;
+    const int bar_xchg = 1 + wg;
     constexpr uint32_t LO = TcK<TC_KC>::LO_OFF;
     constexpr uint32_t A_HALF = 64 * TC_KC * 4 / 16;
     const uint64_t dbase = desc_sw128_base();
     const uint32_t b16 = (smem_u32(b_buf) & 0x3FFFF) >> 4;
     const int q = warp & 3;
-    const int m = q * 32 + lane;
-    uint32_t rowc = 0, phc = 0;
+    uint32_t rowc = 0, phc = 0, exc = 0;
     for (int it = blockIdx.x; it < p.items; it += gridDim.x) {
       const int d = (it / p.hblocks) % p.D;
+      const int b = it / (p.hblocks * p.D);
+      const int h = (it % p.hblocks) * TC_TILES + wg;
+      if (h < p.H && p.residual && p.res_ndhwc)
+        asm volatile("prefetch.global.L2 [%0];" ::"l"(p.residual + ((((size_t)b * p.D + d) * p.H + h) * TC_W + q * 32 + lane) * COUT));
       float acc[2][N3 / 2];
       uint32_t accum = 0;
       for (int kd = 0; kd < 3; ++kd) {
@@ -180,92 +158,21 @@
           }
         }
       }
-      const int h = (it % p.hblocks) * TC_TILES + wg;
       if (h >= p.H) continue;
       const float corr = 1.f + p.kappa * (float)(((d > 0) + 1 + (d + 1 < p.D)) * nchunk * 3 * TcK<TC_KC>::KSTEPS * 3);
-      float out[COUT];
-#pragma unroll
-      for (int pass = 0; pass < C::NPASS; ++pass) {
-        named_bar_sync(bar_stage, 128);
-        tc_stage_pass<COUT>(stage, acc, pass, q, lane);
-        named_bar_sync(bar_stage, 128);
-        const float* srow = stage + m * C::LD;
-        float* xq = xchg + (q + 1) * 2 * TC_PC;
-        if (lane == 31) {
-#pragma unroll
-          for (int i = 0; i < TC_PC; i += 4)
-            *reinterpret_cast<float4*>(xq + i) = *reinterpret_cast<const float4*>(srow + i);
-        }
-        if (lane == 0) {
-#pragma unroll
-          for (int i = 0; i < TC_PC; i += 4)
-            *reinterpret_cast<float4*>(xq + TC_PC + i) = *reinterpret_cast<const float4*>(srow + 2 * TC_PC + i);
-        }
-        named_bar_sync(bar_xchg, 128);
-        const float* xl = xq - 2 * TC_PC;
-        const float* xr = xq + 3 * TC_PC;
-#pragma unroll
-        for (int i0 = 0; i0 < TC_PC; i0 += 4) {
-          const float4 l4 = *reinterpret_cast<const float4*>(xl + i0);
-          const float4 r4 = *reinterpret_cast<const float4*>(xr + i0);
-          const float4 p04 = *reinterpret_cast<const float4*>(srow + i0);
-          const float4 p14 = *reinterpret_cast<const float4*>(srow + TC_PC + i0);
-          const float4 p24 = *reinterpret_cast<const float4*>(srow + 2 * TC_PC + i0);
-          const float le[4] = {l4.x, l4.y, l4.z, l4.w}, re[4] = {r4.x, r4.y, r4.z, r4.w};
-          const float p0[4] = {p04.x, p04.y, p04.z, p04.w}, p1[4] = {p14.x, p14.y, p14.z, p14.w}, p2[4] = {p24.x, p24.y, p24.z, p24.w};
-#pragma unroll
-          for (int k = 0; k < 4; ++k) {
-            float left = __shfl_up_sync(0xffffffffu, p0[k], 1);
-            float right = __shfl_down_sync(0xffffffffu, p2[k], 1);
-            left = (lane == 0) ? le[k] : left;
-            right = (lane == 31) ? re[k] : right;
-            out[pass * TC_PC + i0 + k] = ((left + p1[k]) + right) * corr;
-          }
-        }
-      }
-      const int b = it / (p.hblocks * p.D);
-      const size_t vox = (((size_t)b * p.D + d) * p.H + h) * TC_W + m;
+      frag_unshift<COUT, 1, TC_W>(acc, xchg + (exc & 1) * (C::XCHG_FLOATS / 2), q, lane, corr, bar_xchg);
+      ++exc;
+      const size_t row0 = (((size_t)b * p.D + d) * p.H + h) * TC_W;
       const size_t plane = (size_t)p.D * p.H * TC_W;
-      const size_t ncdhw0 = (size_t)b * p.Cout * plane + ((size_t)d * p.H + h) * TC_W + m;
-      if constexpr (COUT == 32) {
-        if (p.out_ndhwc && (!p.residual || p.res_ndhwc)) {
-          store_ndhwc_chunk32(stage + q * 32 * C::LD, lane, out, p.y + (vox - lane) * COUT,
-                              p.residual ? p.residual + (vox - lane) * COUT : nullptr, COUT, s_scale, s_shift, p.act);
-          continue;
-        }
-      }
-#pragma unroll
-      for (int i = 0; i < COUT; ++i) out[i] = fmaf(out[i], s_scale[i], s_shift[i]);
-      if (p.residual) {
-        if (p.res_ndhwc) {
-          const float4* rp = reinterpret_cast<const float4*>(p.residual + vox * COUT);
-#pragma unroll
-          for (int i = 0; i < COUT / 4; ++i) {
-            const float4 rv = __ldg(rp + i);
-            out[4 * i] += rv.x, out[4 * i + 1] += rv.y, out[4 * i + 2] += rv.z, out[4 * i + 3] += rv.w;
-          }
-        } else {
-#pragma unroll
-          for (int i = 0; i < COUT; ++i)
-            if (i < p.Cout) out[i] += __ldg(p.residual + ncdhw0 + (size_t)i * plane);
-        }
-      }
-      if (p.act == OSB_ACT_RELU) {
-#pragma unroll
-        for (int i = 0; i < COUT; ++i) out[i] = fmaxf(out[i], 0.f);
-      } else if (p.act == OSB_ACT_LEAKY) {
-#pragma unroll
-        for (int i = 0; i < COUT; ++i) out[i] = out[i] > 0.f ? out[i] : 0.01f * out[i];
-      }
-      if (p.out_ndhwc) {
-        float4* yp = reinterpret_cast<float4*>(p.y + vox * COUT);
-#pragma unroll
-        for (int i = 0; i < COUT / 4; ++i) yp[i] = make_float4(out[4 * i], out[4 * i + 1], out[4 * i + 2], out[4 * i + 3]);
-      } else {
-#pragma unroll
-        for (int i = 0; i < COUT; ++i)
-          if (i < p.Cout) p.y[ncdhw0 + (size_t)i * plane] = out[i];
-      }
+      const size_t ncdhw0 = (size_t)b * p.Cout * plane + ((size_t)d * p.H + h) * TC_W;
+      auto rows = [&](int m, ptrdiff_t& yo, ptrdiff_t& ro, ptrdiff_t& go) {
+        yo = p.out_ndhwc ? (ptrdiff_t)(row0 + m) * COUT : (ptrdiff_t)(ncdhw0 + m);
+        ro = p.res_ndhwc ? (ptrdiff_t)(row0 + m) * COUT : (ptrdiff_t)(ncdhw0 + m);
+        go = 0;
+        return true;
+      };
+      frag_epilogue<COUT>(acc, lane, q, tiles + warp * FRAG_TP_FLOATS, s_scale, s_shift, p.act, p.y, p.out_ndhwc ? 1 : plane, p.residual, p.res_ndhwc ? 1 : plane,
+                          nullptr, rows, COUT == 32 ? 32 : p.Cout);
     }
   }
   else if (warp < 4 * TC_WGS + 4) {
diff --git a/openstereo_b200/csrc/conv3d_tcg.cu b/openstereo_b200/csrc/conv3d_tcg.cu
--- a/openstereo_b200/csrc/conv3d_tcg.cu
+++ b/openstereo_b200/csrc/conv3d_tcg.cu
@@ -35,15 +35,15 @@
   static constexpr int NG3 = 3 * G;
   static constexpr int B_SLICE = N3 * ROWB;
   static constexpr int B_SUB = NG3 * ROWB;
-  static constexpr int LD = NG3 + 4;
   static constexpr int NT = TC_WGS * TILES;
   static constexpr int TS = R * DIL;
   static constexpr int HSPAN = NT * TS;
   __host__ __device__ static constexpr int row0(int hb) { return (hb / DIL) * HSPAN + (hb % DIL) * R; }
   __host__ static int hblocks(int H) { return DIL * ((H + HSPAN - 1) / HSPAN); }
   static constexpr int NLW = 4;
-  static constexpr int XCHG_FLOATS = 2 * 4 * 2 * DIL * 32;
-  static constexpr int FIXED_SMEM = 1024 + TC_BSLOTS * 3 * B_SUB + TC_WGS * 128 * LD * 4 + 1024 + TC_WGS * XCHG_FLOATS * 4 + 3 * COUT * 4;
+  static constexpr int XCHG_FLOATS = 2 * frag_xchg_floats<G, DIL>();
+  static constexpr int FIXED_SMEM = 1024 + TC_BSLOTS * 3 * B_SUB + 1024 + TC_WGS * XCHG_FLOATS * 4 + 4 * TC_WGS * FRAG_TP_FLOATS * 4 +
+                                    2 * COUT * 4;
   static constexpr int STAGES = (232448 - FIXED_SMEM) / UNIT_BYTES < 10 ? (232448 - FIXED_SMEM) / UNIT_BYTES : 10;
   static_assert(STAGES >= NLW, "the ring must hold at least one unit per loader warp");
   static constexpr int S_FIRST = -DIL;
@@ -52,10 +52,9 @@
   static constexpr int LO = KC / 8;
   static constexpr int A_OFF = 0;
   static constexpr int B_OFF = A_OFF + STAGES * UNIT_BYTES;
-  static constexpr int STAGE_OFF = B_OFF + TC_BSLOTS * 3 * B_SUB;
-  static constexpr int BAR_OFF = STAGE_OFF + TC_WGS * 128 * LD * 4;
+  static constexpr int BAR_OFF = B_OFF + TC_BSLOTS * 3 * B_SUB;
   static constexpr int THREADS = TC_WG_THREADS;
-  static constexpr size_t SMEM = 1024 + (size_t)BAR_OFF + 1024 + TC_WGS * XCHG_FLOATS * 4 + 3 * COUT * 4;
+  static constexpr size_t SMEM = 1024 + (size_t)BAR_OFF + 1024 + TC_WGS * XCHG_FLOATS * 4 + 4 * TC_WGS * FRAG_TP_FLOATS * 4 + 2 * COUT * 4;
   static_assert(SMEM <= 232448, "shared memory budget of one CTA exceeded");
   static_assert(TILES == 1, "a consumer warpgroup holds one accumulator tile");
   static_assert(DIL == 1 || R == 1, "interleaved row blocks assume one image row per tile");
@@ -90,16 +89,15 @@
   uint8_t* smem = reinterpret_cast<uint8_t*>((reinterpret_cast<uintptr_t>(smem_raw) + 1023) & ~static_cast<uintptr_t>(1023));
   uint8_t* a_buf = smem + C::A_OFF;
   uint8_t* b_buf = smem + C::B_OFF;
-  float* stage = reinterpret_cast<float*>(smem + C::STAGE_OFF);
   uint64_t* bars = reinterpret_cast<uint64_t*>(smem + C::BAR_OFF);
   uint64_t* a_ready = bars;
   uint64_t* a_empty = a_ready + C::STAGES;
   uint64_t* b_full = a_empty + C::STAGES;
   uint64_t* b_empty = b_full + TC_BSLOTS * 3;
   float* xchg = reinterpret_cast<float*>(smem + C::BAR_OFF + 1024);
-  float* s_scale = xchg + TC_WGS * C::XCHG_FLOATS;
+  float* tiles = xchg + TC_WGS * C::XCHG_FLOATS;
+  float* s_scale = tiles + 4 * TC_WGS * FRAG_TP_FLOATS;
   float* s_shift = s_scale + COUT;
-  float* zeros = s_shift + COUT;
 
   const int warp = threadIdx.x >> 5, lane = threadIdx.x & 31;
   const int nchunk = p.Cin / KC;
@@ -121,24 +119,18 @@
   for (int c = threadIdx.x; c < COUT; c += blockDim.x) {
     s_scale[c] = p.scale ? p.scale[c] : 1.f;
     s_shift[c] = p.shift ? p.shift[c] : 0.f;
-    zeros[c] = 0.f;
   }
   __syncthreads();
 
   if (warp < 4 * TC_WGS) {
     setmaxnreg_inc<TC_CONSUMER_REGS>();
     const int wg = warp >> 2;
-    stage += wg * 128 * C::LD;
     xchg += wg * C::XCHG_FLOATS;
-    const int bar_stage = 1 + 2 * wg, bar_xchg = 2 + 2 * wg;
+    const int bar_xchg = 1 + wg;
     const uint64_t dbase = (KC == 32) ? desc_sw128_base() : desc_sw64_base();
     constexpr uint32_t A_HALF = 64 * C::ROWB / 16;
     const uint32_t b16 = (smem_u32(b_buf) & 0x3FFFF) >> 4;
     const int q = warp & 3;
-    const int m = q * 32 + lane;
-    const int rr = m / W, wcol = m % W;
-    const bool has_left_q = ((q * 32) % W) != 0;
-    const bool has_right_q = (((q + 1) * 32) % W) != 0;
     uint32_t unitc = 0, phc = 0, exc = 0;
     for (int it = blockIdx.x; it < p.items; it += gridDim.x) {
       const int cg = (it % C::NG) * C::G;
@@ -147,139 +139,68 @@
       const int hb = (it0 / ctiles) % p.hblocks;
       const int d = (it0 / (ctiles * p.hblocks)) % p.D;
       const int b = it0 / (ctiles * p.hblocks * p.D);
+      auto tile_row = [&](int m, int& h, int& col) {
+        h = C::row0(hb) + wg * C::TS + m / W;
+        col = GW ? ct * C::CSTEP - C::HALO + m : m % W;
+        return h < p.H && (!GW || (m >= C::HALO && m < 128 - C::HALO && col < Wp));
+      };
       {
-        float acc[2][C::NG3 / 2];
-        uint32_t accum = 0;
-        for (int kd = 0; kd < 3; ++kd) {
-          const int din = d + kd - 1;
-          if (din < 0 || din >= p.D) continue;
-          for (int ch = 0; ch < nchunk; ++ch, ++phc) {
-#pragma unroll
-            for (int s = C::S_FIRST; s <= C::S_LAST; ++s) {
-              if (!C::used(s)) continue;
-              const uint32_t slot = unitc % C::STAGES, par = (unitc / C::STAGES) & 1;
-              mbar_wait(&a_ready[slot], par);
-              const uint64_t da0 = dbase | (uint64_t)((smem_u32(a_buf + slot * C::UNIT_BYTES) & 0x3FFFF) >> 4);
-#pragma unroll
-              for (int kh = 0; kh < 3; ++kh) {
-                if (C::tile_of(s, kh) != wg) continue;
-                const uint32_t bslot = (phc & 1) * 3 + kh;
-                mbar_wait(&b_full[bslot], (phc >> 1) & 1);
-                const uint64_t db0 = dbase | (uint64_t)(b16 + (bslot * C::B_SUB) / 16);
-                wg_fence();
-#pragma unroll
-                for (int ks = 0; ks < C::KSTEPS; ++ks)
-                  wg_mma_split<C::NG3>(acc, da0 + 2 * ks, A_HALF, db0 + 2 * ks, C::LO, ks > 0 ? 1u : accum);
-                wg_commit();
-                wg_wait_all();
-                accum = 1;
-                wg_release(&b_empty[bslot], lane);
-              }
-              wg_release(&a_empty[slot], lane);
-              ++unitc;
+        int h, col;
+        if (tile_row(q * 32 + lane, h, col)) {
+          const ptrdiff_t vox = (((ptrdiff_t)b * p.D + d) * p.H + h) * Wp + col;
+          if (p.residual && p.res_ndhwc) asm volatile("prefetch.global.L2 [%0];" ::"l"(p.residual + vox * YS + cg));
+          if (GATE && p.gate) asm volatile("prefetch.global.L2 [%0];" ::"l"(p.gate + (((ptrdiff_t)b * p.H + h) * Wp + col) * YS + cg));
+        }
+      }
+      float acc[2][C::NG3 / 2];
+      uint32_t accum = 0;
+      for (int kd = 0; kd < 3; ++kd) {
+        const int din = d + kd - 1;
+        if (din < 0 || din >= p.D) continue;
+        for (int ch = 0; ch < nchunk; ++ch, ++phc) {
+#pragma unroll
+          for (int s = C::S_FIRST; s <= C::S_LAST; ++s) {
+            if (!C::used(s)) continue;
+            const uint32_t slot = unitc % C::STAGES, par = (unitc / C::STAGES) & 1;
+            mbar_wait(&a_ready[slot], par);
+            const uint64_t da0 = dbase | (uint64_t)((smem_u32(a_buf + slot * C::UNIT_BYTES) & 0x3FFFF) >> 4);
+#pragma unroll
+            for (int kh = 0; kh < 3; ++kh) {
+              if (C::tile_of(s, kh) != wg) continue;
+              const uint32_t bslot = (phc & 1) * 3 + kh;
+              mbar_wait(&b_full[bslot], (phc >> 1) & 1);
+              const uint64_t db0 = dbase | (uint64_t)(b16 + (bslot * C::B_SUB) / 16);
+              wg_fence();
+#pragma unroll
+              for (int ks = 0; ks < C::KSTEPS; ++ks)
+                wg_mma_split<C::NG3>(acc, da0 + 2 * ks, A_HALF, db0 + 2 * ks, C::LO, ks > 0 ? 1u : accum);
+              wg_commit();
+              wg_wait_all();
+              accum = 1;
+              wg_release(&b_empty[bslot], lane);
             }
+            wg_release(&a_empty[slot], lane);
+            ++unitc;
           }
         }
-        named_bar_sync(bar_stage, 128);
-        wg_stage<C::NG3>(stage, C::LD, acc, q, lane);
-        named_bar_sync(bar_stage, 128);
-      }
-      const int col = GW ? ct * C::CSTEP - C::HALO + m : wcol;
-      const bool cvalid = !GW || (m >= C::HALO && m < 128 - C::HALO && col < Wp);
-      const uint32_t vmask = GW ? __ballot_sync(0xffffffffu, cvalid) : 0xffffffffu;
+      }
       const float corr = 1.f + p.kappa * (float)(((d > 0) + 1 + (d + 1 < p.D)) * nchunk * 3 * C::KSTEPS * 3);
-      {
-        const int h = C::row0(hb) + wg * C::TS + rr;
-        const bool live = h < p.H;
+      frag_unshift<C::G, DIL, W>(acc, xchg + (exc & 1) * (C::XCHG_FLOATS / 2), q, lane, corr, bar_xchg);
+      ++exc;
+      const size_t plane = (size_t)p.D * p.H * Wp;
+      auto rows = [&](int m, ptrdiff_t& yo, ptrdiff_t& ro, ptrdiff_t& go) {
+        int h, col;
+        const bool ok = tile_row(m, h, col);
         const ptrdiff_t vox = (((ptrdiff_t)b * p.D + d) * p.H + h) * Wp + col;
-        if (live && cvalid && p.residual && p.res_ndhwc) {
-          const float* rp = p.residual + vox * YS;
-#pragma unroll
-          for (int k = 0; k < COUT; k += 32) asm volatile("prefetch.global.L2 [%0];" ::"l"(rp + k));
-        }
-        const size_t plane = (size_t)p.D * p.H * Wp;
-        const ptrdiff_t ncdhw0 = (ptrdiff_t)b * COUT * plane + ((ptrdiff_t)d * p.H + h) * Wp + col;
-        {
-          const float* srow = stage + m * C::LD;
-          float* xb = xchg + (exc & 1) * (4 * 2 * DIL * 32);
-          ++exc;
-          if (lane >= 32 - DIL) {
-#pragma unroll
-            for (int i = 0; i < 32; i += 4)
-              *reinterpret_cast<float4*>(xb + ((q * 2) * DIL + lane - (32 - DIL)) * 32 + i) = *reinterpret_cast<const float4*>(srow + i);
-          }
-          if (lane < DIL) {
-#pragma unroll
-            for (int i = 0; i < 32; i += 4)
-              *reinterpret_cast<float4*>(xb + ((q * 2 + 1) * DIL + lane) * 32 + i) = *reinterpret_cast<const float4*>(srow + 2 * C::G + i);
-          }
-          named_bar_sync(bar_xchg, 128);
-          const float* xl = has_left_q ? xb + (((q - 1) * 2) * DIL + (lane < DIL ? lane : 0)) * 32 : zeros;
-          const float* xr = has_right_q ? xb + (((q + 1) * 2 + 1) * DIL + (lane >= 32 - DIL ? lane - (32 - DIL) : 0)) * 32 : zeros;
-          float out[32];
-#pragma unroll
-          for (int i0 = 0; i0 < 32; i0 += 4) {
-            const float4 l4 = *reinterpret_cast<const float4*>(xl + i0);
-            const float4 r4 = *reinterpret_cast<const float4*>(xr + i0);
-            const float4 p04 = *reinterpret_cast<const float4*>(srow + i0);
-            const float4 p14 = *reinterpret_cast<const float4*>(srow + C::G + i0);
-            const float4 p24 = *reinterpret_cast<const float4*>(srow + 2 * C::G + i0);
-            const float le[4] = {l4.x, l4.y, l4.z, l4.w}, re[4] = {r4.x, r4.y, r4.z, r4.w};
-            const float p0[4] = {p04.x, p04.y, p04.z, p04.w}, p1[4] = {p14.x, p14.y, p14.z, p14.w}, p2[4] = {p24.x, p24.y, p24.z, p24.w};
-#pragma unroll
-            for (int k = 0; k < 4; ++k) {
-              const int i = i0 + k;
-              float left = __shfl_up_sync(0xffffffffu, p0[k], DIL);
-              float right = __shfl_down_sync(0xffffffffu, p2[k], DIL);
-              left = (lane < DIL) ? le[k] : left;
-              right = (lane >= 32 - DIL) ? re[k] : right;
-              if (W < 32) {
-                left = (wcol < DIL) ? 0.f : left;
-                right = (wcol >= W - DIL) ? 0.f : right;
-              }
-              out[i] = ((left + p1[k]) + right) * corr;
-            }
-          }
-          const uint32_t vm = (W < 32) ? __ballot_sync(0xffffffffu, live) : (live ? vmask : 0u);
-          if (vm && p.out_ndhwc && (!p.residual || p.res_ndhwc)) {
-            const ptrdiff_t gvox = GATE ? ((ptrdiff_t)b * p.H + h) * Wp + col - lane : 0;
-            store_ndhwc_chunk32(stage + q * 32 * C::LD, lane, out, p.y + (vox - lane) * YS + cg,
-                                p.residual ? p.residual + (vox - lane) * YS + cg : nullptr, YS, s_scale + cg, s_shift + cg, p.act,
-                                vm, (GATE && p.gate) ? p.gate + gvox * YS + cg : nullptr);
-          } else if (live && cvalid) {
-#pragma unroll
-            for (int i = 0; i < 32; ++i) out[i] = fmaf(out[i], s_scale[cg + i], s_shift[cg + i]);
-            if (p.residual) {
-              if (p.res_ndhwc) {
-                const float4* rp = reinterpret_cast<const float4*>(p.residual + vox * YS + cg);
-#pragma unroll
-                for (int i = 0; i < 8; ++i) {
-                  const float4 rv = __ldg(rp + i);
-                  out[4 * i] += rv.x, out[4 * i + 1] += rv.y, out[4 * i + 2] += rv.z, out[4 * i + 3] += rv.w;
-                }
-              } else {
-#pragma unroll
-                for (int i = 0; i < 32; ++i) out[i] += __ldg(p.residual + ncdhw0 + (size_t)(cg + i) * plane);
-              }
-            }
-            if (p.act == OSB_ACT_RELU) {
-#pragma unroll
-              for (int i = 0; i < 32; ++i) out[i] = fmaxf(out[i], 0.f);
-            } else if (p.act == OSB_ACT_LEAKY) {
-#pragma unroll
-              for (int i = 0; i < 32; ++i) out[i] = out[i] > 0.f ? out[i] : 0.01f * out[i];
-            }
-            if (p.out_ndhwc) {
-              float4* yp = reinterpret_cast<float4*>(p.y + vox * YS + cg);
-#pragma unroll
-              for (int i = 0; i < 8; ++i) yp[i] = make_float4(out[4 * i], out[4 * i + 1], out[4 * i + 2], out[4 * i + 3]);
-            } else {
-#pragma unroll
-              for (int i = 0; i < 32; ++i) p.y[ncdhw0 + (size_t)(cg + i) * plane] = out[i];
-            }
-          }
-        }
-      }
+        const ptrdiff_t ncdhw = (ptrdiff_t)b * COUT * plane + ((ptrdiff_t)d * p.H + h) * Wp + col;
+        yo = p.out_ndhwc ? vox * YS : ncdhw;
+        ro = p.res_ndhwc ? vox * YS : ncdhw;
+        go = (((ptrdiff_t)b * p.H + h) * Wp + col) * YS;
+        return ok;
+      };
+      frag_epilogue<C::G>(acc, lane, q, tiles + warp * FRAG_TP_FLOATS, s_scale + cg, s_shift + cg, p.act, p.y + (p.out_ndhwc ? (size_t)cg : cg * plane),
+                          p.out_ndhwc ? 1 : plane, p.residual ? p.residual + (p.res_ndhwc ? (size_t)cg : cg * plane) : nullptr,
+                          p.res_ndhwc ? 1 : plane, (GATE && p.gate) ? p.gate + cg : nullptr, rows, C::G);
     }
   }
   else if (warp < 4 * TC_WGS + C::NLW) {
diff --git a/openstereo_b200/csrc/tc_common.cuh b/openstereo_b200/csrc/tc_common.cuh
--- a/openstereo_b200/csrc/tc_common.cuh
+++ b/openstereo_b200/csrc/tc_common.cuh
@@ -216,6 +216,176 @@
   static constexpr int LO_OFF = KC / 8;
 };
 
+template <int G, int DIL>
+constexpr int frag_xchg_floats() { return 8 * 2 * DIL * G; }
+template <int G, int DIL, int W>
+__device__ __forceinline__ void frag_unshift(float (&acc)[2][3 * G / 2], float* xb, int wq, int lane, float corr, int bar) {
+  constexpr int SIDE = DIL * G;
+  const int l4 = lane >> 2, c0 = 2 * (lane & 3);
+#pragma unroll
+  for (int h = 0; h < 2; ++h) {
+    float* grp = xb + (4 * h + wq) * 2 * SIDE;
+    if (l4 >= 8 - DIL) {
+#pragma unroll
+      for (int j = 0; j < G / 8; ++j)
+        *reinterpret_cast<float2*>(grp + (l4 - 8 + DIL) * G + 8 * j + c0) = make_float2(acc[h][4 * j + 2], acc[h][4 * j + 3]);
+    }
+    if (l4 < DIL) {
+#pragma unroll
+      for (int j = 0; j < G / 8; ++j)
+        *reinterpret_cast<float2*>(grp + SIDE + l4 * G + 8 * j + c0) =
+            make_float2(acc[h][4 * (j + G / 4)], acc[h][4 * (j + G / 4) + 1]);
+    }
+  }
+  named_bar_sync(bar, 128);
+  const int src_l = (lane - 4 * DIL) & 31, src_r = (lane + 4 * DIL) & 31;
+  const bool wrap_l = l4 >= 8 - DIL, wrap_r = l4 < DIL;
+#pragma unroll
+  for (int h = 0; h < 2; ++h) {
+    const int g = 4 * h + wq;
+    const float* xl = xb + (g > 0 ? g - 1 : 0) * 2 * SIDE + (l4 < DIL ? l4 : 0) * G + c0;
+    const float* xr = xb + (g < 7 ? g + 1 : 7) * 2 * SIDE + SIDE + (l4 >= 8 - DIL ? l4 - 8 + DIL : 0) * G + c0;
+    const int mlo = (64 * h + 16 * wq + l4) % W, mhi = (64 * h + 16 * wq + 8 + l4) % W;
+#pragma unroll
+    for (int j = 0; j < G / 8; ++j) {
+      const float2 sl = *reinterpret_cast<const float2*>(xl + 8 * j);
+      const float2 sr = *reinterpret_cast<const float2*>(xr + 8 * j);
+#pragma unroll
+      for (int c2 = 0; c2 < 2; ++c2) {
+        const float p0lo = acc[h][4 * j + c2], p0hi = acc[h][4 * j + 2 + c2];
+        const float p2lo = acc[h][4 * (j + G / 4) + c2], p2hi = acc[h][4 * (j + G / 4) + 2 + c2];
+        float llo = __shfl_sync(0xffffffffu, p0lo, src_l);
+        float lhi = __shfl_sync(0xffffffffu, wrap_l ? p0lo : p0hi, src_l);
+        float rlo = __shfl_sync(0xffffffffu, wrap_r ? p2hi : p2lo, src_r);
+        float rhi = __shfl_sync(0xffffffffu, p2hi, src_r);
+        llo = (l4 < DIL) ? (c2 ? sl.y : sl.x) : llo;
+        rhi = (l4 >= 8 - DIL) ? (c2 ? sr.y : sr.x) : rhi;
+        llo = (mlo < DIL) ? 0.f : llo;
+        lhi = (mhi < DIL) ? 0.f : lhi;
+        rlo = (mlo >= W - DIL) ? 0.f : rlo;
+        rhi = (mhi >= W - DIL) ? 0.f : rhi;
+        float& olo = acc[h][4 * (j + G / 8) + c2];
+        float& ohi = acc[h][4 * (j + G / 8) + 2 + c2];
+        olo = ((llo + olo) + rlo) * corr;
+        ohi = ((lhi + ohi) + rhi) * corr;
+      }
+    }
+  }
+}
+constexpr int FRAG_TP_STRIDE = 40;
+constexpr int FRAG_TP_FLOATS = 16 * FRAG_TP_STRIDE;
+template <int G, class Rows>
+__device__ __forceinline__ void frag_epilogue(const float (&acc)[2][3 * G / 2], int lane, int wq, float* tbuf, const float* sc,
+                                              const float* sh, int act, float* y, size_t ycs, const float* res, size_t rcs,
+                                              const float* gate, Rows rows, int nch) {
+  const int c0 = 2 * (lane & 3), l4 = lane >> 2;
+  if constexpr (G == 32) {
+    if (ycs == 1 && (!res || rcs == 1)) {
+      const int c4 = 4 * (lane & 7), sub = lane >> 3;
+      const float4 a = *reinterpret_cast<const float4*>(sc + c4);
+      const float4 b = *reinterpret_cast<const float4*>(sh + c4);
+#pragma unroll
+      for (int h = 0; h < 2; ++h) {
+        __syncwarp();
+#pragma unroll
+        for (int j = 0; j < 4; ++j)
+#pragma unroll
+          for (int rh = 0; rh < 2; ++rh)
+            *reinterpret_cast<float2*>(tbuf + (8 * rh + l4) * FRAG_TP_STRIDE + 8 * j + c0) =
+                make_float2(acc[h][4 * (j + 4) + 2 * rh], acc[h][4 * (j + 4) + 2 * rh + 1]);
+        __syncwarp();
+        float4 o[4];
+        ptrdiff_t yo[4], ro[4], go[4];
+        bool ok[4];
+#pragma unroll
+        for (int i = 0; i < 4; ++i) {
+          ok[i] = rows(64 * h + 16 * wq + 4 * i + sub, yo[i], ro[i], go[i]);
+          o[i] = *reinterpret_cast<const float4*>(tbuf + (4 * i + sub) * FRAG_TP_STRIDE + c4);
+          o[i].x = fmaf(o[i].x, a.x, b.x), o[i].y = fmaf(o[i].y, a.y, b.y), o[i].z = fmaf(o[i].z, a.z, b.z), o[i].w = fmaf(o[i].w, a.w, b.w);
+        }
+        if (res) {
+          float4 r[4];
+#pragma unroll
+          for (int i = 0; i < 4; ++i) r[i] = ok[i] ? __ldg(reinterpret_cast<const float4*>(res + ro[i] + c4)) : make_float4(0.f, 0.f, 0.f, 0.f);
+#pragma unroll
+          for (int i = 0; i < 4; ++i) o[i].x += r[i].x, o[i].y += r[i].y, o[i].z += r[i].z, o[i].w += r[i].w;
+        }
+        if (act == OSB_ACT_RELU) {
+#pragma unroll
+          for (int i = 0; i < 4; ++i) o[i].x = fmaxf(o[i].x, 0.f), o[i].y = fmaxf(o[i].y, 0.f), o[i].z = fmaxf(o[i].z, 0.f), o[i].w = fmaxf(o[i].w, 0.f);
+        } else if (act == OSB_ACT_LEAKY) {
+#pragma unroll
+          for (int i = 0; i < 4; ++i) {
+            o[i].x = o[i].x > 0.f ? o[i].x : 0.01f * o[i].x, o[i].y = o[i].y > 0.f ? o[i].y : 0.01f * o[i].y;
+            o[i].z = o[i].z > 0.f ? o[i].z : 0.01f * o[i].z, o[i].w = o[i].w > 0.f ? o[i].w : 0.01f * o[i].w;
+          }
+        }
+        if (gate) {
+          float4 g[4];
+#pragma unroll
+          for (int i = 0; i < 4; ++i) g[i] = ok[i] ? __ldg(reinterpret_cast<const float4*>(gate + go[i] + c4)) : make_float4(1.f, 1.f, 1.f, 1.f);
+#pragma unroll
+          for (int i = 0; i < 4; ++i) o[i].x *= g[i].x, o[i].y *= g[i].y, o[i].z *= g[i].z, o[i].w *= g[i].w;
+        }
+#pragma unroll
+        for (int i = 0; i < 4; ++i)
+          if (ok[i]) *reinterpret_cast<float4*>(y + yo[i] + c4) = o[i];
+      }
+      return;
+    }
+  }
+#pragma unroll
+  for (int h = 0; h < 2; ++h) {
+    float2 rv[G / 8][2], gv[G / 8][2];
+#pragma unroll
+    for (int j = 0; j < G / 8; ++j)
+#pragma unroll
+      for (int rh = 0; rh < 2; ++rh) {
+        const int c = 8 * j + c0;
+        ptrdiff_t yo, ro, go;
+        const bool live = rows(64 * h + 16 * wq + l4 + 8 * rh, yo, ro, go);
+        rv[j][rh] = make_float2(0.f, 0.f);
+        gv[j][rh] = make_float2(1.f, 1.f);
+        if (res) {
+          if (rcs == 1) {
+            if (live) rv[j][rh] = __ldg(reinterpret_cast<const float2*>(res + ro + c));
+          } else {
+            if (live && c < nch) rv[j][rh].x = __ldg(res + ro + (size_t)c * rcs);
+            if (live && c + 1 < nch) rv[j][rh].y = __ldg(res + ro + (size_t)(c + 1) * rcs);
+          }
+        }
+        if (gate && live) gv[j][rh] = __ldg(reinterpret_cast<const float2*>(gate + go + c));
+      }
+#pragma unroll
+    for (int j = 0; j < G / 8; ++j) {
+      const int c = 8 * j + c0;
+      const float2 a = *reinterpret_cast<const float2*>(sc + c);
+      const float2 b = *reinterpret_cast<const float2*>(sh + c);
+#pragma unroll
+      for (int rh = 0; rh < 2; ++rh) {
+        ptrdiff_t yo, ro, go;
+        const bool live = rows(64 * h + 16 * wq + l4 + 8 * rh, yo, ro, go);
+        float v0 = fmaf(acc[h][4 * (j + G / 8) + 2 * rh], a.x, b.x);
+        float v1 = fmaf(acc[h][4 * (j + G / 8) + 2 * rh + 1], a.y, b.y);
+        if (res) v0 += rv[j][rh].x, v1 += rv[j][rh].y;
+        if (act == OSB_ACT_RELU) {
+          v0 = fmaxf(v0, 0.f), v1 = fmaxf(v1, 0.f);
+        } else if (act == OSB_ACT_LEAKY) {
+          v0 = v0 > 0.f ? v0 : 0.01f * v0, v1 = v1 > 0.f ? v1 : 0.01f * v1;
+        }
+        if (gate) v0 *= gv[j][rh].x, v1 *= gv[j][rh].y;
+        if (!live) continue;
+        if (ycs == 1) {
+          *reinterpret_cast<float2*>(y + yo + c) = make_float2(v0, v1);
+        } else {
+          if (c < nch) y[yo + (size_t)c * ycs] = v0;
+          if (c + 1 < nch) y[yo + (size_t)(c + 1) * ycs] = v1;
+        }
+      }
+    }
+  }
+}
+
 constexpr int TP_STRIDE = 36;
 constexpr int TP_WARP_FLOATS = 32 * TP_STRIDE;
 
```

New measurement: 283.7, median of 6. +6.8%, better.
